# anonymousauthors001/SGS-GNN

Measured on AMD Instinct MI355X. Metric: sampled edges/sec + training steps/sec, Reddit hybrid 20% sparsity, higher is better.
Workload: dtype f32

## Files before the change

include/sgs_hip.h:

```cpp
#ifndef SGS_HIP_H_
#define SGS_HIP_H_

#include <stddef.h>
#include <stdint.h>

#ifdef __cplusplus
extern "C" {
#endif

#define SGS_ABI_VERSION 1

#define SGS_OK 0
#define SGS_EINVAL (-1)
#define SGS_EWORKSPACE (-2)
#define SGS_EHIP (-3)

typedef void* sgs_stream_t;

int sgs_abi_version(void);
const char* sgs_last_error(void);

int sgs_rng_set_epoch_buffer(const uint64_t* epoch_dev);
int sgs_exp_noise(uint64_t seed, uint64_t stream_id, int64_t E, float* noise, sgs_stream_t stream);
int sgs_dropout_keep(uint64_t seed, uint32_t site, int64_t rows, int64_t cols, float p, uint8_t* keep,
// ... 8 lines not shown
#define SGS_SAMPLE_PRIOR 1

size_t sgs_sample_topq_workspace_bytes(int64_t E);
int sgs_sample_topq(int mode, const float* p, const float* prior, double degree_bias_coef,
                    const float* noise, uint64_t seed, uint64_t stream_id, int64_t E, int64_t q,
                    const int64_t* edge_index, uint8_t* mask, int64_t* sampled_eid,
                    int64_t* sampled_edge_index, float* sampled_p, float* stats, float* keys_out,
                    void* ws, size_t ws_bytes, sgs_stream_t stream);

size_t sgs_sample_topq_cover_workspace_bytes(int64_t E, int64_t N);
int sgs_sample_topq_cover_variant(int64_t N, int64_t E);
int sgs_sample_topq_cover(int mode, const float* p, const float* prior, double degree_bias_coef, const float* noise,
                          uint64_t seed, uint64_t stream_id, int64_t E, int64_t q, const int64_t* edge_index,
                          int64_t N, const int32_t* in_ptr, const int32_t* in_src, const int32_t* in_eid,
                          uint8_t* mask, int64_t* sampled_eid, int64_t* sampled_edge_index, float* sampled_p,
                          float* stats, float* keys_out, int32_t* cover_info, void* ws, size_t ws_bytes, sgs_stream_t stream);

int sgs_gather_columns(const int64_t* edge_index, int64_t E, const int64_t* idx, int64_t q, int64_t* out, sgs_stream_t stream);

size_t sgs_sampler_shard_workspace_bytes(int64_t E_local);
int64_t sgs_sampler_chunk(void);
int sgs_sampler_shard_partials(int stage, const float* p, int64_t E, const float* scal, float* part, sgs_stream_t stream);
int sgs_sampler_shard_finalize(int stage, const float* part_all, int64_t nblk_all, float* scal, sgs_stream_t stream);
int sgs_sampler_shard_keys(int mode, const float* p, const float* prior, double degree_bias_coef, const float* noise,
                           uint64_t seed, uint64_t stream_id, int64_t edge_offset, int64_t E, const float* scal,
                           uint32_t* keys, float* keys_out, uint32_t* hist, sgs_stream_t stream);
int sgs_sampler_shard_hist(const uint32_t* keys, int64_t E, int pass, const void* state, uint32_t* hist,
                           sgs_stream_t stream);
int sgs_sampler_select(uint32_t* hist, int pass, int64_t q, void* state, sgs_stream_t stream);
int sgs_sampler_shard_count(const uint32_t* keys, int64_t E, const void* state, uint32_t* counts, void* ws,
                            size_t ws_bytes, sgs_stream_t stream);
int sgs_sampler_shard_compact(const uint32_t* keys, int64_t E, const void* state, int64_t ties_local, int64_t q_local,
                              int64_t edge_offset, const float* p, const int64_t* edge_index_local, uint8_t* mask,
                              int64_t* sampled_eid, int64_t* sampled_edge_index, float* sampled_p, void* ws,
                              size_t ws_bytes, sgs_stream_t stream);

int sgs_st_weights_fwd(const float* p, const float* prior, double degree_bias_coef, const float* stats,
                       const int64_t* sampled_eid, int64_t E, int64_t q, float* w, sgs_stream_t stream);
size_t sgs_st_weights_bwd_workspace_bytes(int64_t E, int64_t q);
int sgs_st_weights_bwd(const float* p, const float* prior, double degree_bias_coef, const float* stats,
                       const int64_t* sampled_eid, const float* grad_w, int64_t E, int64_t q, float* grad_p,
                       void* ws, size_t ws_bytes, sgs_stream_t stream);

size_t sgs_graph_build_workspace_bytes(int64_t n_edges, int64_t N);
int sgs_graph_build(const int64_t* edge_index, int64_t n_edges, int64_t N, int32_t* in_ptr, int32_t* in_src,
                    int32_t* in_eid, int32_t* out_ptr, int32_t* out_dst, int32_t* out_eid, int32_t* loop_eid,
                    void* ws, size_t ws_bytes, sgs_stream_t stream);

size_t sgs_graph_filter_workspace_bytes(int64_t E_parent, int64_t N);
int sgs_graph_filter(const int32_t* pin_ptr, const int32_t* pin_src, const int32_t* pin_eid, const int32_t* pout_ptr,
                     const int32_t* pout_dst, const int32_t* pout_eid, int64_t E_parent, int64_t N, const uint8_t* mask,
                     const int64_t* sampled_eid, int64_t q, int32_t* in_ptr, int32_t* in_src, int32_t* in_eid, int32_t* out_ptr,
                     int32_t* out_dst, int32_t* out_eid, int32_t* loop_eid, void* ws, size_t ws_bytes, sgs_stream_t stream);

size_t sgs_graph_build_src_sorted_workspace_bytes(int64_t n_edges, int64_t N);
int sgs_graph_build_src_sorted(const int64_t* edge_index, int64_t n_edges, int64_t N, int32_t* in_ptr, int32_t* in_src, int32_t* in_eid,
                               int32_t* out_ptr, int32_t* out_dst, int32_t* out_eid, int32_t* loop_eid, int32_t* unsorted, void* ws,
                               size_t ws_bytes, sgs_stream_t stream);

int sgs_gcn_norm_fwd(const float* w, int64_t n_edges, int64_t N, const int32_t* in_ptr, const int32_t* in_src,
                     const int32_t* in_eid, const int32_t* out_ptr, const int32_t* out_dst, const int32_t* out_eid,
                     const int32_t* loop_eid, float* dis, float* loopw, float* what_in, float* what_out,
                     float* what_loop, sgs_stream_t stream);

int sgs_gcn_degree_partial(const float* w, int64_t n_edges, int64_t N, const int32_t* in_ptr, const int32_t* in_src,
                           const int32_t* in_eid, float* degpart, sgs_stream_t stream);
int sgs_gcn_norm_from_degree(const float* w, const float* degsum, int64_t n_edges, int64_t N, const int32_t* in_ptr,
                             const int32_t* in_src, const int32_t* in_eid, const int32_t* out_ptr,
                             const int32_t* out_dst, const int32_t* out_eid, float* dis, float* loopw, float* what_in,
                             float* what_out, float* what_loop, sgs_stream_t stream);
int sgs_bias_act(const float* X, const float* bias, int64_t N, int64_t D, int act, float p_drop, uint64_t seed,
                 uint32_t site, float* Y, sgs_stream_t stream);
int sgs_bias_act_rows(const float* X, const float* bias, int64_t n_rows, int64_t D, int64_t row_offset, int act, float p_drop,
                      uint64_t seed, uint32_t site, float* Y, sgs_stream_t stream);

int sgs_mean_weights(int64_t n_edges, int64_t N, const int32_t* in_ptr, const int32_t* out_ptr, const int32_t* out_dst,
                     float* what_in, float* what_out, sgs_stream_t stream);
int sgs_degree_prior_logits(const int64_t* edge_index, int64_t E, int64_t N, const int32_t* in_ptr,
                            const int32_t* out_ptr, float* logits, sgs_stream_t stream);

size_t sgs_gcn_norm_bwd_workspace_bytes(int64_t N);
int sgs_gcn_norm_bwd(const float* w, const float* gw_hat, const float* gloop, int64_t n_edges, int64_t N,
                     const float* dis, const float* loopw, const int32_t* in_ptr, const int32_t* in_src,
                     const int32_t* in_eid, const int32_t* out_ptr, const int32_t* out_dst, const int32_t* out_eid,
                     const int32_t* loop_eid, const int64_t* edge_index, float* dw, void* ws, size_t ws_bytes,
                     sgs_stream_t stream);
int sgs_gcn_norm_bwd_sum(const float* w, const float* gw_hat, const float* gloop, const float* gw_hat2, const float* gloop2, const float* dw_add,
                         int64_t n_edges, int64_t N, const float* dis, const float* loopw, const int32_t* in_ptr, const int32_t* in_src,
                         const int32_t* in_eid, const int32_t* out_ptr, const int32_t* out_dst, const int32_t* out_eid,
                         const int32_t* loop_eid, const int64_t* edge_index, float* dw, void* ws, size_t ws_bytes, sgs_stream_t stream);

int sgs_gcn_norm_bwd_node(const float* w, const float* gw_hat, const float* gloop, int64_t n_edges, int64_t N,
                          const float* dis, const float* loopw, const int32_t* in_ptr, const int32_t* in_src,
                          const int32_t* in_eid, const int32_t* out_ptr, const int32_t* out_dst, const int32_t* out_eid,
                          float* Hn, sgs_stream_t stream);
int sgs_gcn_norm_bwd_edge(const float* gw_hat, const float* gloop, int64_t n_edges, int64_t N, const float* dis,
                          const int32_t* loop_eid, const int64_t* edge_index, const float* Hn, float* dw,
                          sgs_stream_t stream);

#define SGS_ACT_NONE 0
#define SGS_ACT_RELU 1
#define SGS_ACT_RELU_DROPOUT 2
int sgs_spmm_csr(const float* X, int64_t N, int64_t D, int64_t nnz, const int32_t* ptr, const int32_t* col, const float* val,
                 const float* diag, const float* bias, int act, float p_drop, uint64_t seed, uint32_t site, float* Y,
                 sgs_stream_t stream);

int sgs_sddmm_csr(const float* A, const float* B, int64_t N, int64_t D, int64_t nnz, const int32_t* ptr, const int32_t* col,
                  const int32_t* eid, float* g, float* gdiag, sgs_stream_t stream);

int sgs_spmm_csr_variant(int64_t N, int64_t D, int64_t nnz, int aligned16);
int sgs_sddmm_csr_variant(int64_t N, int64_t D, int64_t nnz, int aligned16);

int sgs_spmm_long_rows_set(int on);
int sgs_spmm_long_rows_threshold(void);
int sgs_spmm_long_rows_active(int64_t N, int64_t D);

// ... 90 lines not shown
                                    float* out_codes, float* out_U, float* out_U_raw, sgs_stream_t stream);
int sgs_edge_score_bwd_prep_sd_pack(const float* codes, int64_t N, int64_t H, const int64_t* edge_index, int64_t E, const int64_t* active_eid,
                                    int64_t n_active, const float* grad_p, const float* p, const uint32_t* maskbits, float* dz, uint32_t* dvbits,
                                    int32_t* sd, const float* W1, const float* w2, float p_drop, void* ws, size_t ws_bytes, sgs_stream_t stream);
int sgs_edge_score_bwd_dfeat_fused_packed(const uint32_t* dvbits, const float* dz, const int32_t* sd, const float* codes, int64_t n, int64_t N,
                                          int64_t H, float* G, float* opart, const void* ws, size_t ws_bytes, sgs_stream_t stream);
int sgs_edge_score_bwd_core_bits(const float* codes, const float* U, int64_t N, int64_t H, const int64_t* edge_index, int64_t E,
                                 int64_t edge_id_offset, const int64_t* active_eid, int64_t n_active, const float* grad_p, const float* W1,
                                 const float* b1, const float* w2, const float* b2, float p_drop, uint64_t seed, uint32_t site,
                                 uint32_t* dvbits, float* hdz_part, float* dz, float* feat, void* ws, size_t ws_bytes, sgs_stream_t stream);
int sgs_edge_score_bwd_dfeat_bits(const uint32_t* dvbits, const float* dz, int64_t n, int64_t H, const float* W1, const float* w2, float p_drop,
                                  float* dfeat, void* ws, size_t ws_bytes, sgs_stream_t stream);
int sgs_endpoint_reduce_pair_bits(const float* dfeat, const uint32_t* dvbits, const float* dz, const float* w2, float p_drop, const float* codes,
                                  int64_t N, int64_t H, int64_t nnz, const int32_t* in_ptr, const int32_t* in_src, const int32_t* in_eid,
                                  const int32_t* out_ptr, const int32_t* out_dst, const int32_t* out_eid, float* out_codes, float* out_U,
                                  float* out_U_raw, sgs_stream_t stream);
int sgs_gemm_tn_mask_supported(int64_t K, int64_t M, int64_t N);
int sgs_gemm_tn_mask_gather(const uint32_t* Abits, const float* dz, const float* rowscale, float scale, const float* codes, int64_t codes_rows,
                            const int32_t* sd, int64_t K, int64_t M, int64_t N, float* C, int64_t ldc, float* colsum_A, float* dz_sum, float* C_raw,
                            float* colsum_raw, void* ws, size_t ws_bytes, sgs_stream_t stream);
void sgs_gemm_tn_set_gather_variant(int shared, int slabs);
int sgs_gemm_tn_mask(const uint32_t* Abits, const float* dz, const float* rowscale, float scale, const float* B, int64_t K, int64_t M, int64_t N,
                     float* C, int64_t ldc, float* colsum_A, float* dz_sum, float* C_raw, float* colsum_raw, void* ws, size_t ws_bytes,
                     sgs_stream_t stream);

int sgs_edge_score_bf16_supported(int64_t H);
int sgs_edge_score_fwd_bf16(const float* codes, const float* U, int64_t N, int64_t H, const int64_t* edge_index, int64_t E,
                            int64_t edge_id_offset, const float* W1, const float* b1, const float* w2, const float* b2, float p_drop,
                            uint64_t seed, uint32_t site, float* p_out, void* ws, size_t ws_bytes, sgs_stream_t stream);
int sgs_edge_score_fwd_paired_bf16(const float* codes, const float* U, int64_t N, int64_t H, const int64_t* edge_index, int64_t E,
                                   int64_t edge_id_offset, const int32_t* canon, int64_t M, const int32_t* mate, const float* W1, const float* b1,
                                   const float* w2, const float* b2, float p_drop, uint64_t seed, uint32_t site, float* p_out, void* ws,
                                   size_t ws_bytes, sgs_stream_t stream);
int sgs_edge_score_fwd_mask_bf16(const float* codes, const float* U, int64_t N, int64_t H, const int64_t* edge_index, int64_t E,
                                 int64_t edge_id_offset, const int32_t* canon, int64_t M, const int32_t* mate, const float* W1, const float* b1,
                                 const float* w2, const float* b2, float p_drop, uint64_t seed, uint32_t site, float* p_out, uint32_t* maskbits,
                                 void* ws, size_t ws_bytes, sgs_stream_t stream);
int sgs_edge_score_bwd_dfeat_bits_bf16(const uint32_t* dvbits, const float* dz, int64_t n, int64_t H, const float* W1, const float* w2,
                                       float p_drop, float* dfeat, void* ws, size_t ws_bytes, sgs_stream_t stream);
int sgs_edge_score_bwd_prep_sd_pack_bf16(const float* codes, int64_t N, int64_t H, const int64_t* edge_index, int64_t E, const int64_t* active_eid,
                                         int64_t n_active, const float* grad_p, const float* p, const uint32_t* maskbits, float* dz, uint32_t* dvbits,
                                         int32_t* sd, const float* W1, const float* w2, float p_drop, void* ws, size_t ws_bytes, sgs_stream_t stream);
int sgs_edge_score_bwd_dfeat_fused_bf16(const uint32_t* dvbits, const float* dz, const int32_t* sd, const float* codes, int64_t n, int64_t N,
                                        int64_t H, const float* W1, const float* w2, float p_drop, float* G, float* opart, void* ws, size_t ws_bytes,
                                        sgs_stream_t stream);
int sgs_edge_score_bwd_dfeat_fused_packed_bf16(const uint32_t* dvbits, const float* dz, const int32_t* sd, const float* codes, int64_t n, int64_t N,
                                               int64_t H, float* G, float* opart, const void* ws, size_t ws_bytes, sgs_stream_t stream);
int sgs_gemm_tn_mask_bf16(const uint32_t* Abits, const float* dz, const float* rowscale, float scale, const float* B, int64_t K, int64_t M, int64_t N,
                          float* C, int64_t ldc, float* colsum_A, float* dz_sum, float* C_raw, float* colsum_raw, void* ws, size_t ws_bytes,
                          sgs_stream_t stream);
int sgs_gemm_tn_mask_gather_bf16(const uint32_t* Abits, const float* dz, const float* rowscale, float scale, const float* codes, int64_t codes_rows,
                                 const int32_t* sd, int64_t K, int64_t M, int64_t N, float* C, int64_t ldc, float* colsum_A, float* dz_sum, float* C_raw,
                                 float* colsum_raw, void* ws, size_t ws_bytes, sgs_stream_t stream);

int sgs_endpoint_reduce(const float* M_out, const float* M_in, const float* T, int64_t N, int64_t H, int64_t nnz,
                        const int32_t* in_ptr, const int32_t* in_src, const int32_t* in_eid, const int32_t* out_ptr,
                        const int32_t* out_dst, const int32_t* out_eid, float sign_out, float sign_in, float* out,
                        sgs_stream_t stream);
int sgs_endpoint_reduce_pair(const float* dfeat, const float* dv, const float* codes, int64_t N, int64_t H, int64_t nnz,
                             const int32_t* in_ptr, const int32_t* in_src, const int32_t* in_eid, const int32_t* out_ptr,
                             const int32_t* out_dst, const int32_t* out_eid, float* out_codes, float* out_U, sgs_stream_t stream);

int sgs_masked_correct(const float* logits, int64_t N, int64_t C, const int64_t* y, const uint8_t* train_mask,
                       int32_t* correct, sgs_stream_t stream);
int sgs_masked_correct_pair(const float* logits_a, const float* logits_b, int64_t N, int64_t C, const int64_t* y,
                            const uint8_t* train_mask, int32_t* correct4, sgs_stream_t stream);

int sgs_confusion_counts(const float* logits, int64_t N, int64_t C, const int64_t* y, const uint8_t* m0, const uint8_t* m1, const uint8_t* m2,
                         int64_t* conf, sgs_stream_t stream);
int sgs_confusion_variant(int64_t N, int64_t C);
int sgs_confusion_variant_set(int code);

size_t sgs_gate_counts_workspace_bytes(int64_t N);
int sgs_gate_counts(const float* logits_a, const float* logits_b, int64_t N, int64_t C, const int64_t* y, const uint8_t* train_mask,
                    int32_t* out5, const uint64_t* seq_dev, int32_t* dst_host_mapped, void* ws, size_t ws_bytes, sgs_stream_t stream);

int sgs_loss_tick(float* loss_sum, const float* loss, uint64_t* epoch, sgs_stream_t stream);
int sgs_publish_to_host(const int32_t* src_dev, int64_t n, const uint64_t* seq_dev, int32_t* dst_host_mapped, sgs_stream_t stream);

int sgs_masked_ce_fwd(const float* logits, int64_t N, int64_t C, const int64_t* y, const uint8_t* train_mask,
                      float* loss, float* row_lse, float* rowloss, int32_t* n_rows, sgs_stream_t stream);
int sgs_masked_ce_bwd(const float* logits, int64_t N, int64_t C, const int64_t* y, const uint8_t* train_mask,
                      const float* row_lse, const int32_t* n_rows, const float* grad_loss, float* dlogits,
                      sgs_stream_t stream);

size_t sgs_edge_reg_workspace_bytes(int64_t q);
int sgs_edge_reg_fwd(const float* w, const int64_t* sampled_edge_index, int64_t q, const float* logits, int64_t N,
                     int64_t C, const int64_t* y, const uint8_t* train_mask, float coef1, float coef2, float* out,
                     float* cos_out, void* ws, size_t ws_bytes, sgs_stream_t stream);
int sgs_edge_reg_bwd(const float* w, const int64_t* sampled_edge_index, int64_t q, int64_t q_global, const float* logits,
                     int64_t N, int64_t C, const int64_t* y, const uint8_t* train_mask, const float* out, float coef1,
                     float coef2, const float* grad_loss, float* dw, float* Gs, float* Gd, sgs_stream_t stream);

int sgs_hybrid_loss_fwd(const float* logits, int64_t N, int64_t C, const int64_t* y, const uint8_t* train_mask, const float* w,
                        const int64_t* sampled_edge_index, int64_t q, float coef1, float coef2, float* out, float* row_lse, float* rowloss,
                        int32_t* n_rows, void* ws, size_t ws_bytes, sgs_stream_t stream);
int sgs_masked_ce_bwd_acc(const float* logits, int64_t N, int64_t C, const int64_t* y, const uint8_t* train_mask, const float* row_lse,
                          const int32_t* n_rows, const float* grad_loss, float* dlogits, sgs_stream_t stream);

int sgs_masked_ce_w_fwd(const float* logits, int64_t N, int64_t C, const int64_t* y, const uint8_t* train_mask, const float* weight,
                        float label_smoothing, float* loss, float* row_lse, float* rowloss, float* den, sgs_stream_t stream);
int sgs_masked_ce_w_bwd(const float* logits, int64_t N, int64_t C, const int64_t* y, const uint8_t* train_mask, const float* weight,
                        float label_smoothing, const float* row_lse, const float* den, const float* grad_loss, float* dlogits,
                        sgs_stream_t stream);
int sgs_masked_ce_w_bwd_acc(const float* logits, int64_t N, int64_t C, const int64_t* y, const uint8_t* train_mask, const float* weight,
                            float label_smoothing, const float* row_lse, const float* den, const float* grad_loss, float* dlogits,
// ... 208 lines not shown
```

sgs-gnn_amd/csrc/edge_score.hip:

```cpp
#include <type_traits>

#include "sgs_common.h"
#include "endpoint_reduce.h"

namespace sgs {
namespace {

constexpr int kT = 256;
constexpr int kBM = 64;
constexpr int kBK = 16;
using f32x16 = __attribute__((ext_vector_type(16))) float;

__global__ void __launch_bounds__(kT) transpose_w1a(const float* __restrict__ W1, int H, float* __restrict__ WaT) {
    __shared__ float t[32][33];
    const int bx = blockIdx.x * 32, by = blockIdx.y * 32;
    const int tx = threadIdx.x & 31, ty = threadIdx.x >> 5;
    for (int r = ty; r < 32; r += 8) {
        const int h = by + r, k = bx + tx;
        t[r][tx] = (h < H && k < H) ? W1[static_cast<int64_t>(h) * 2 * H + k] : 0.f;
    }
    __syncthreads();
    for (int r = ty; r < 32; r += 8) {
        const int k = bx + r, h = by + tx;
        if (k < H && h < H) WaT[static_cast<int64_t>(k) * H + h] = t[tx][r];
    }
}

__global__ void __launch_bounds__(kT) transpose_w1_full(const float* __restrict__ W1, int H, float* __restrict__ WT) {
    __shared__ float t[32][33];
    const int bx = blockIdx.x * 32, by = blockIdx.y * 32;
    const int tx = threadIdx.x & 31, ty = threadIdx.x >> 5;
    for (int r = ty; r < 32; r += 8) {
        const int h = by + r, k = bx + tx;
        t[r][tx] = (h < H && k < 2 * H) ? W1[static_cast<int64_t>(h) * 2 * H + k] : 0.f;
    }
    __syncthreads();
    for (int r = ty; r < 32; r += 8) {
        const int k = bx + r, h = by + tx;
        if (k < 2 * H && h < H) WT[static_cast<int64_t>(k) * H + h] = t[tx][r];
    }
}

struct ScoreArgs {
    const float* codes;
    const float* U;
    const int64_t* src;
    const int64_t* dst;
    const int64_t* active;
    int64_t n;
    const int32_t* canon;
    const int32_t* mate;
    const int64_t* dyn_n;
    int64_t row_offset;
    int H;
    const float* WaT;
    const float* b1;
// ... 1738 lines not shown
                    ok[u] = k < total ? 1.f : 0.f;
                    sg[u] = k < total ? (isout ? 1.f : -1.f) : 0.f;
                }
                float m1[kEpU][4], m2[kEpU][4], t[kEpU][4];
                uint32_t wd[kEpU];
                float dzr[kEpU];
#pragma unroll
                for (int u = 0; u < kEpU; ++u) {
                    *reinterpret_cast<float4*>(m1[u]) = *reinterpret_cast<const float4*>(dfeat + static_cast<int64_t>(er[u]) * H + c0);
                    *reinterpret_cast<float4*>(t[u]) = *reinterpret_cast<const float4*>(codes + static_cast<int64_t>(cr[u]) * H + c0);
                    if constexpr (BITS) {
                        wd[u] = bits[static_cast<int64_t>(er[u]) * (H >> 5) + (c0 >> 5)];
                        dzr[u] = dz[er[u]];
                    } else {
                        *reinterpret_cast<float4*>(m2[u]) = *reinterpret_cast<const float4*>(dv + static_cast<int64_t>(er[u]) * H + c0);
                    }
                }
#pragma unroll
                for (int u = 0; u < kEpU; ++u) {
                    if constexpr (BITS) {
                        const uint32_t w = wd[u] >> (c0 & 31);
#pragma unroll
                        for (int j = 0; j < 4; ++j) m2[u][j] = (w >> j) & 1u ? dzr[u] : 0.f;
                    }
#pragma unroll
                    for (int j = 0; j < 4; ++j) {
                        a1[j] = fmaf(ok[u] * m1[u][j], t[u][j], a1[j]);
                        a2[j] = fmaf(sg[u], m2[u][j], a2[j]);
                    }
                }
            }
        }
#pragma unroll
        for (int j = 0; j < 4; ++j) { part[0][wave][lane * 4 + j] = a1[j]; part[1][wave][lane * 4 + j] = a2[j]; }
        __syncthreads();
        for (int tt = threadIdx.x; tt < 512; tt += 64 * NW) {
            const int which = tt >> 8, c = tt & 255;
            if (cbase + c < H) {
                float sum = 0.f;
#pragma unroll
                for (int g = 0; g < NW; g += 4) sum += (part[which][g][c] + part[which][g + 1][c]) + (part[which][g + 2][c] + part[which][g + 3][c]);
                if (BITS && which) {
                    if (out_Uraw) out_Uraw[v * H + cbase + c] = sum;
                    sum *= w2[cbase + c] * scale;
                }
                (which ? out_U : out_codes)[v * H + cbase + c] = sum;
            }
        }
        __syncthreads();
    }
}

template <int NW>
__global__ void __launch_bounds__(64 * NW) scorer_bwd_reduce(const float* __restrict__ G, const float* __restrict__ opart,
                                                            const uint32_t* __restrict__ bits, const float* __restrict__ dz,
                                                            const float* __restrict__ w2, float scale, int64_t N, int64_t H,
                                                            const int* __restrict__ in_ptr, const int* __restrict__ in_eid,
                                                            const int* __restrict__ out_ptr, float* __restrict__ out_codes,
                                                            float* __restrict__ out_U, float* __restrict__ out_Uraw) {
    __shared__ float part[2][NW][256];
    const int lane = threadIdx.x & 63, wave = threadIdx.x >> 6;
    const int64_t v = blockIdx.x;
    const int ob = out_ptr[v], no = out_ptr[v + 1] - ob;
    const int ib = in_ptr[v], ni = in_ptr[v + 1] - ib;
    const int w0 = ob >> 5, np = no > 0 ? ((ob + no - 1) >> 5) - w0 + 1 : 0;
    const int wpr = static_cast<int>(H >> 5);
    for (int64_t cbase = 0; cbase < H; cbase += 256) {
        const int64_t c0 = cbase + static_cast<int64_t>(lane) * 4;
        float a1[4] = {0.f, 0.f, 0.f, 0.f}, a2[4] = {0.f, 0.f, 0.f, 0.f};
        if (c0 < H) {
            const int wsel = static_cast<int>(c0 >> 5), wsh = static_cast<int>(c0 & 31);
            for (int k0 = wave; k0 < ni; k0 += kEpU * NW) {
                int er[kEpU];
                float ok[kEpU];
#pragma unroll
                for (int u = 0; u < kEpU; ++u) {
                    const int k = k0 + NW * u;
                    er[u] = in_eid[ib + (k < ni ? k : ni - 1)];
                    ok[u] = k < ni ? 1.f : 0.f;
                }
                float4 m1[kEpU];
                uint32_t wd[kEpU];
                float dzr[kEpU];
#pragma unroll
                for (int u = 0; u < kEpU; ++u) {
                    m1[u] = *reinterpret_cast<const float4*>(G + static_cast<int64_t>(er[u]) * H + c0);
                    wd[u] = bits[static_cast<int64_t>(er[u]) * wpr + wsel];
                    dzr[u] = dz[er[u]];
                }
#pragma unroll
                for (int u = 0; u < kEpU; ++u) {
                    const uint32_t w = wd[u] >> wsh;
                    const float dd = ok[u] * dzr[u];
                    a1[0] = fmaf(ok[u], m1[u].x, a1[0]); a1[1] = fmaf(ok[u], m1[u].y, a1[1]);
                    a1[2] = fmaf(ok[u], m1[u].z, a1[2]); a1[3] = fmaf(ok[u], m1[u].w, a1[3]);
#pragma unroll
                    for (int j = 0; j < 4; ++j) a2[j] -= (w >> j) & 1u ? dd : 0.f;
                }
            }
            for (int k0 = wave; k0 < no; k0 += kEpU * NW) {
                uint32_t wd[kEpU];
                float dzr[kEpU];
#pragma unroll
                for (int u = 0; u < kEpU; ++u) {
                    const int k = k0 + NW * u;
                    const int64_t e = ob + (k < no ? k : no - 1);
                    wd[u] = bits[e * wpr + wsel];
                    dzr[u] = dz[e] * (k < no ? 1.f : 0.f);
                }
#pragma unroll
                for (int u = 0; u < kEpU; ++u) {
                    const uint32_t w = wd[u] >> wsh;
#pragma unroll
                    for (int j = 0; j < 4; ++j) a2[j] += (w >> j) & 1u ? dzr[u] : 0.f;
                }
            }
            for (int k0 = wave; k0 < np; k0 += kEpU * NW) {
                float4 m1[kEpU];
                float ok[kEpU];
#pragma unroll
                for (int u = 0; u < kEpU; ++u) {
                    const int k = k0 + NW * u;
                    const int64_t slot = static_cast<int64_t>(w0 + (k < np ? k : np - 1)) + v;
                    m1[u] = *reinterpret_cast<const float4*>(opart + slot * H + c0);
                    ok[u] = k < np ? 1.f : 0.f;
                }
#pragma unroll
                for (int u = 0; u < kEpU; ++u) {
                    a1[0] = fmaf(ok[u], m1[u].x, a1[0]); a1[1] = fmaf(ok[u], m1[u].y, a1[1]);
                    a1[2] = fmaf(ok[u], m1[u].z, a1[2]); a1[3] = fmaf(ok[u], m1[u].w, a1[3]);
                }
            }
        }
#pragma unroll
        for (int j = 0; j < 4; ++j) { part[0][wave][lane * 4 + j] = a1[j]; part[1][wave][lane * 4 + j] = a2[j]; }
        __syncthreads();
        for (int tt = threadIdx.x; tt < 512; tt += 64 * NW) {
            const int which = tt >> 8, c = tt & 255;
            if (cbase + c < H) {
                float sum = 0.f;
#pragma unroll
                for (int g = 0; g < NW; g += 4) sum += (part[which][g][c] + part[which][g + 1][c]) + (part[which][g + 2][c] + part[which][g + 3][c]);
                if (which) {
                    if (out_Uraw) out_Uraw[v * H + cbase + c] = sum;
                    sum *= w2[cbase + c] * scale;
                }
                (which ? out_U : out_codes)[v * H + cbase + c] = sum;
            }
        }
        __syncthreads();
    }
}

__global__ void __launch_bounds__(256) epd_endpoint_reduce(const float* __restrict__ dfeat2, const float* __restrict__ A, int64_t N, int64_t H,
                                                          const int* __restrict__ in_ptr, const int* __restrict__ in_src,
                                                          const int* __restrict__ in_eid, const int* __restrict__ out_ptr,
                                                          const int* __restrict__ out_dst, const int* __restrict__ out_eid,
                                                          const int64_t* __restrict__ active, int64_t row_offset, uint64_t seed_x, uint32_t site_x,
                                                          uint64_t seed_y, uint32_t site_y, const uint64_t* __restrict__ epoch, uint32_t thresh,
                                                          float scale, int use_drop, float* __restrict__ dA) {
    constexpr int NW = 4;
    __shared__ float part[NW][256];
    const int lane = threadIdx.x & 63, wave = threadIdx.x >> 6;
    const int64_t v = blockIdx.x;
    const int ob = out_ptr[v], no = out_ptr[v + 1] - ob;
    const int ib = in_ptr[v], ni = in_ptr[v + 1] - ib;
    const int total = no + ni;
    const uint64_t sx = fold_epoch(seed_x, epoch), sy = fold_epoch(seed_y, epoch);
    for (int64_t cbase = 0; cbase < H; cbase += 256) {
        const int64_t c0 = cbase + static_cast<int64_t>(lane) * 4;
        float acc[4] = {0.f, 0.f, 0.f, 0.f};
        if (c0 < H) {
            for (int k = wave; k < total; k += NW) {
                const bool isout = k < no;
                const int idx = isout ? ob + k : ib + (k - no);
                const int r = (isout ? out_eid : in_eid)[idx];
                const int o = (isout ? out_dst : in_src)[idx];
                const int64_t e = row_offset + (active ? active[r] : static_cast<int64_t>(r));
                const float4 fa = *reinterpret_cast<const float4*>(dfeat2 + static_cast<int64_t>(r) * 2 * H + c0);
                const float4 fb = *reinterpret_cast<const float4*>(dfeat2 + static_cast<int64_t>(r) * 2 * H + H + c0);
                const float4 ao = *reinterpret_cast<const float4*>(A + static_cast<int64_t>(o) * H + c0);
                float ko[4] = {1.f, 1.f, 1.f, 1.f}, km[4] = {1.f, 1.f, 1.f, 1.f};
                if (use_drop) {
                    const uint32_t rx = dropout_row_key(sx, site_x, static_cast<uint64_t>(e)), ry = dropout_row_key(sy, site_y, static_cast<uint64_t>(e));
                    const uint32_t rmine = isout ? rx : ry, rother = isout ? ry : rx;
                    const uint32_t m0 = dropout_pair_bits(rmine, static_cast<uint32_t>(c0 >> 1)), m1 = dropout_pair_bits(rmine, static_cast<uint32_t>((c0 >> 1) + 1));
                    const uint32_t o0 = dropout_pair_bits(rother, static_cast<uint32_t>(c0 >> 1)), o1 = dropout_pair_bits(rother, static_cast<uint32_t>((c0 >> 1) + 1));
                    km[0] = (m0 & 0xFFFFu) >= thresh ? scale : 0.f; km[1] = (m0 >> 16) >= thresh ? scale : 0.f;
                    km[2] = (m1 & 0xFFFFu) >= thresh ? scale : 0.f; km[3] = (m1 >> 16) >= thresh ? scale : 0.f;
                    ko[0] = (o0 & 0xFFFFu) >= thresh ? scale : 0.f; ko[1] = (o0 >> 16) >= thresh ? scale : 0.f;
                    ko[2] = (o1 & 0xFFFFu) >= thresh ? scale : 0.f; ko[3] = (o1 >> 16) >= thresh ? scale : 0.f;
                }
                const float fav[4] = {fa.x, fa.y, fa.z, fa.w}, fbv[4] = {fb.x, fb.y, fb.z, fb.w}, aov[4] = {ao.x, ao.y, ao.z, ao.w};
                const float sg = isout ? 1.f : -1.f;
#pragma unroll
                for (int j = 0; j < 4; ++j) acc[j] += (fav[j] * (aov[j] * ko[j]) + sg * fbv[j]) * km[j];
            }
        }
#pragma unroll
        for (int j = 0; j < 4; ++j) part[wave][lane * 4 + j] = acc[j];
        __syncthreads();
        const int tt = threadIdx.x;
        if (cbase + tt < H) dA[v * H + cbase + tt] = (part[0][tt] + part[1][tt]) + (part[2][tt] + part[3][tt]);
        __syncthreads();
// ... 570 lines not shown
    if (n == 0) return SGS_OK;
    SGS_REQUIRE(dvbits && dz && sd && codes && (packed || (W1 && w2)) && G && opart, SGS_EINVAL, "%s: null pointer", who);
    SGS_REQUIRE(ws && ws_bytes >= sgs_edge_score_workspace_bytes(0, H, 0), SGS_EWORKSPACE, "%s: workspace too small", who);
    uint4* const Wp16 = fused_wp16(ws, H);
    if (!packed) launch_pack_w1a<true>(P, W1, H, Wp16, stream, w2, 1.0f / (1.0f - p_drop));
    ScoreArgs a{};
    a.inbits = dvbits; a.indz = dz; a.n = n; a.H = static_cast<int>(H); a.feat = G; a.codes = codes; a.sd = sd; a.opart = opart;
    return P == 1 ? launch_bf16x6<5, 1>(a, Wp16, n, H, stream) : launch_bf16x6<5, 3>(a, Wp16, n, H, stream);
}

int sgs_edge_score_bwd_dfeat_fused(const uint32_t* dvbits, const float* dz, const int32_t* sd, const float* codes, int64_t n, int64_t N, int64_t H,
                                   const float* W1, const float* w2, float p_drop, float* G, float* opart, void* ws, size_t ws_bytes,
                                   sgs_stream_t stream_) {
    return bwd_dfeat_fused_impl("sgs_edge_score_bwd_dfeat_fused", 3, sgs_edge_score_bwd_bits_supported, false, dvbits, dz, sd, codes, n, N, H, W1, w2,
                                p_drop, G, opart, ws, ws_bytes, stream_);
}

int sgs_edge_score_bwd_dfeat_fused_packed(const uint32_t* dvbits, const float* dz, const int32_t* sd, const float* codes, int64_t n, int64_t N,
                                          int64_t H, float* G, float* opart, const void* ws, size_t ws_bytes, sgs_stream_t stream_) {
    return bwd_dfeat_fused_impl("sgs_edge_score_bwd_dfeat_fused_packed", 3, sgs_edge_score_bwd_bits_supported, true, dvbits, dz, sd, codes, n, N, H,
                                nullptr, nullptr, 0.f, G, opart, const_cast<void*>(ws), ws_bytes, stream_);
}

int sgs_edge_score_bwd_dfeat_fused_bf16(const uint32_t* dvbits, const float* dz, const int32_t* sd, const float* codes, int64_t n, int64_t N,
                                        int64_t H, const float* W1, const float* w2, float p_drop, float* G, float* opart, void* ws, size_t ws_bytes,
                                        sgs_stream_t stream_) {
    return bwd_dfeat_fused_impl("sgs_edge_score_bwd_dfeat_fused_bf16", 1, sgs_edge_score_bf16_supported, false, dvbits, dz, sd, codes, n, N, H, W1, w2,
                                p_drop, G, opart, ws, ws_bytes, stream_);
}

int sgs_edge_score_bwd_dfeat_fused_packed_bf16(const uint32_t* dvbits, const float* dz, const int32_t* sd, const float* codes, int64_t n, int64_t N,
                                               int64_t H, float* G, float* opart, const void* ws, size_t ws_bytes, sgs_stream_t stream_) {
    return bwd_dfeat_fused_impl("sgs_edge_score_bwd_dfeat_fused_packed_bf16", 1, sgs_edge_score_bf16_supported, true, dvbits, dz, sd, codes, n, N, H,
                                nullptr, nullptr, 0.f, G, opart, const_cast<void*>(ws), ws_bytes, stream_);
}

int sgs_edge_score_bwd_reduce_fused(const float* G, const float* opart, const uint32_t* dvbits, const float* dz, const float* w2, float p_drop,
                                    int64_t N, int64_t H, int64_t nnz, const int32_t* in_ptr, const int32_t* in_eid, const int32_t* out_ptr,
                                    float* out_codes, float* out_U, float* out_U_raw, sgs_stream_t stream_) {
    hipStream_t stream = static_cast<hipStream_t>(stream_);
    SGS_REQUIRE(N >= 0 && H >= 0 && H % 32 == 0 && N < (int64_t(1) << 31) && p_drop >= 0.f && p_drop < 1.f, SGS_EINVAL,
                "sgs_edge_score_bwd_reduce_fused: needs H %% 32 == 0");
    if (N == 0 || H == 0) return SGS_OK;
    SGS_REQUIRE(G && opart && dvbits && dz && w2 && in_ptr && in_eid && out_ptr && out_codes && out_U, SGS_EINVAL,
                "sgs_edge_score_bwd_reduce_fused: null pointer");
    const dim3 grid(static_cast<unsigned>(N));
    const float scale = 1.0f / (1.0f - p_drop);
    SGS_LAUNCH_ROWBLOCK((scorer_bwd_reduce<16>), (scorer_bwd_reduce<4>), G, opart, dvbits, dz, w2, scale, N, H, in_ptr, in_eid, out_ptr, out_codes,
                        out_U, out_U_raw);
    SGS_LAUNCH_OK();
    return SGS_OK;
}

int sgs_edge_score_dw2_from_parts(const float* W1, const float* T_raw, const float* U, const float* R_raw, const float* b1, const float* c_raw,
                                  int64_t N, int64_t H, float p_drop, float* dw2, sgs_stream_t stream_) {
    hipStream_t stream = static_cast<hipStream_t>(stream_);
    SGS_REQUIRE(N > 0 && H > 0 && p_drop >= 0.f && p_drop < 1.f && W1 && T_raw && U && R_raw && b1 && c_raw && dw2, SGS_EINVAL,
                "sgs_edge_score_dw2_from_parts: bad arguments");
    hipLaunchKernelGGL(scorer_dw2_from_parts, dim3(static_cast<unsigned>(H)), dim3(kT), 0, stream, W1, T_raw, U, R_raw, b1, c_raw, N,
                       static_cast<int>(H), 1.0f / (1.0f - p_drop), dw2);
    SGS_LAUNCH_OK();
    return SGS_OK;
}

int sgs_endpoint_reduce_pair_bits(const float* dfeat, const uint32_t* dvbits, const float* dz, const float* w2, float p_drop, const float* codes,
                                  int64_t N, int64_t H, int64_t nnz, const int32_t* in_ptr, const int32_t* in_src, const int32_t* in_eid,
                                  const int32_t* out_ptr, const int32_t* out_dst, const int32_t* out_eid, float* out_codes, float* out_U,
                                  float* out_U_raw, sgs_stream_t stream_) {
    hipStream_t stream = static_cast<hipStream_t>(stream_);
    SGS_REQUIRE(N >= 0 && H >= 0 && H % 32 == 0 && N < (int64_t(1) << 31) && p_drop >= 0.f && p_drop < 1.f, SGS_EINVAL,
                "sgs_endpoint_reduce_pair_bits: needs H %% 32 == 0");
    if (N == 0 || H == 0) return SGS_OK;
    SGS_REQUIRE(dfeat && dvbits && dz && w2 && codes && in_ptr && out_ptr && out_codes && out_U, SGS_EINVAL,
                "sgs_endpoint_reduce_pair_bits: null pointer");
    const dim3 grid(static_cast<unsigned>(N));
    const float scale = 1.0f / (1.0f - p_drop);
    const float* nodv = nullptr;
    SGS_LAUNCH_ROWBLOCK((endpoint_reduce_pair_rowblock<16, true>), (endpoint_reduce_pair_rowblock<4, true>), dfeat, nodv, codes, N, H, in_ptr, in_src,
                        in_eid, out_ptr, out_dst, out_eid, out_codes, out_U, dvbits, dz, w2, scale, out_U_raw);
    SGS_LAUNCH_OK();
    return SGS_OK;
}

size_t sgs_edge_score_epd_workspace_bytes(int64_t H) { return carve_bytes(2 * static_cast<size_t>(H < 0 ? 0 : H) * (H < 0 ? 0 : H), 4) + 256; }

static int epd_args(ScoreArgs& a, const char* who, const float* A, int64_t N, int64_t H, const int64_t* edge_index, int64_t E, const int64_t* active,
                    int64_t n, int64_t edge_id_offset, const float* W1, const float* b1, const float* w2, const float* b2, float p_hidden, uint64_t seed,
                    uint32_t site, float p_ep,
                    uint64_t seed_x, uint32_t site_x, uint64_t seed_y, uint32_t site_y, void* ws, size_t ws_bytes, hipStream_t stream) {
    if (int rc = check_common(who, N, H, E, p_hidden)) return rc;
    SGS_REQUIRE(H % 16 == 0, SGS_EINVAL, "%s: the endpoint-dropout scorer needs H %% 16 == 0 (H=%lld)", who, (long long)H);
    SGS_REQUIRE(p_ep >= 0.f && p_ep < 1.f, SGS_EINVAL, "%s: bad endpoint dropout probability", who);
    SGS_REQUIRE(A && edge_index && W1 && b1 && w2 && b2, SGS_EINVAL, "%s: null pointer", who);
    SGS_REQUIRE(ws && ws_bytes >= sgs_edge_score_epd_workspace_bytes(H), SGS_EWORKSPACE, "%s: workspace too small", who);
    Carver cv(ws);
    float* WT = cv.take<float>(2 * static_cast<size_t>(H) * H);
    hipLaunchKernelGGL(transpose_w1_full, dim3(cdiv(2 * H, 32), cdiv(H, 32)), dim3(kT), 0, stream, W1, static_cast<int>(H), WT);
    score_args(a, A, nullptr, edge_index, E, active, n, edge_id_offset, H, WT, b1, w2, b2, p_hidden, seed, site);
    a.epd = p_ep > 0.f; a.seed_x = seed_x; a.seed_y = seed_y; a.site_x = site_x; a.site_y = site_y;
    a.ep_scale = 1.0f / (1.0f - p_ep); a.ep_thresh = dropout_thresh(p_ep);
    return SGS_OK;
}

int sgs_edge_score_epd_fwd(const float* A, int64_t N, int64_t H, const int64_t* edge_index, int64_t E, int64_t edge_id_offset, const float* W1,
                           const float* b1, const float* w2, const float* b2, float p_hidden, uint64_t seed, uint32_t site, float p_ep,
                           uint64_t seed_x, uint32_t site_x, uint64_t seed_y, uint32_t site_y, float* p_out, void* ws, size_t ws_bytes,
// ... 57 lines not shown
```

sgs-gnn_amd/csrc/gcn.hip:

```cpp
#include "sgs_common.h"

namespace sgs {
size_t graph_sort_workspace_bytes(int64_t n, int64_t N);
size_t graph_src_sorted_workspace_bytes(int64_t n, int64_t N);
int graph_build_src_sorted(const int64_t* ei, int64_t n, int64_t N, int32_t* in_ptr, int32_t* in_src, int32_t* in_eid, int32_t* out_ptr,
                           int32_t* out_dst, int32_t* out_eid, int32_t* loop_eid, int32_t* unsorted_flag, void* ws, size_t ws_bytes,
                           hipStream_t stream);
int graph_build_by_sort(const int64_t* ei, int64_t n, int64_t N, int32_t* in_ptr, int32_t* in_src, int32_t* in_eid, int32_t* out_ptr,
                        int32_t* out_dst, int32_t* out_eid, int32_t* loop_eid, void* ws, size_t ws_bytes, hipStream_t stream);
}

namespace sgs {
namespace {

constexpr int kT = 256;
constexpr int kMaxLdsRow = 8192;

__global__ void __launch_bounds__(kT) count_degrees(const int64_t* __restrict__ ei, int64_t n_edges, int* __restrict__ cnt_in,
                                                   int* __restrict__ cnt_out, int* __restrict__ loop_eid) {
    const int64_t e = static_cast<int64_t>(blockIdx.x) * kT + threadIdx.x;
    if (e >= n_edges) return;
    const int s = static_cast<int>(ei[e]), d = static_cast<int>(ei[n_edges + e]);
    atomicAdd(&cnt_in[d], 1);
    atomicAdd(&cnt_out[s], 1);
// ... 213 lines not shown
        if (e < E && mask[e]) v |= 1u << j;
    }
    bits[w] = v;
}
template <bool BITS>
__device__ __forceinline__ bool mask_at(const uint8_t* __restrict__ mask, int e) {
    if (BITS) return (reinterpret_cast<const uint32_t*>(mask)[e >> 5] >> (e & 31)) & 1u;
    return mask[e] != 0;
}

template <bool BITS>
__device__ __forceinline__ void filter_count_scatter_body(const int* __restrict__ in_ptr, const int* __restrict__ in_eid,
                                                          const int* __restrict__ out_ptr, const int* __restrict__ out_eid, int64_t N,
                                                          const uint8_t* __restrict__ mask, const int64_t* __restrict__ sampled_eid,
                                                          int64_t q, int64_t n_row_blocks, int* __restrict__ cnt_in,
                                                          int* __restrict__ cnt_out, int* __restrict__ pos, int64_t nrows) {
    if (static_cast<int64_t>(blockIdx.x) >= n_row_blocks) {
        const int64_t j = (static_cast<int64_t>(blockIdx.x) - n_row_blocks) * kT + threadIdx.x;
        if (j < q) pos[sampled_eid[j]] = static_cast<int>(j);
        return;
    }
    const int lane = threadIdx.x & 63;
    const int64_t r = (static_cast<int64_t>(blockIdx.x) * kT + threadIdx.x) >> 6;
    if (r >= nrows) return;
    const bool out = r >= N;
    const int64_t row = out ? r - N : r;
    const int* ptr = out ? out_ptr : in_ptr;
    const int* eid = out ? out_eid : in_eid;
    int c = 0;
    const int b = ptr[row], e = ptr[row + 1];
    for (int k = b + lane; k < e; k += 256) {
        int id[4];
#pragma unroll
        for (int u = 0; u < 4; ++u) id[u] = eid[min(k + 64 * u, e - 1)];
#pragma unroll
        for (int u = 0; u < 4; ++u) {
            const bool m = mask_at<BITS>(mask, id[u]);
            c += (k + 64 * u < e && m) ? 1 : 0;
        }
    }
    c = wave_sum_int_all(c);
    if (lane == 0) (out ? cnt_out : cnt_in)[row] = c;
}
template <bool BITS>
__global__ void __launch_bounds__(kT) filter_count_scatter(const int* __restrict__ in_ptr, const int* __restrict__ in_eid,
                                                          const int* __restrict__ out_ptr, const int* __restrict__ out_eid, int64_t N,
                                                          const uint8_t* __restrict__ mask, const int64_t* __restrict__ sampled_eid,
                                                          int64_t q, int64_t n_row_blocks, int* __restrict__ cnt_in,
                                                          int* __restrict__ cnt_out, int* __restrict__ pos) {
    filter_count_scatter_body<BITS>(in_ptr, in_eid, out_ptr, out_eid, N, mask, sampled_eid, q, n_row_blocks, cnt_in, cnt_out, pos, 2 * N);
}

constexpr int64_t kSelfScanRows = 4096;
template <bool BITS, bool SCAN>
__device__ __forceinline__ void filter_fill_body(int64_t nrows, const int* __restrict__ pin_ptr, const int* __restrict__ pin_src, const int* __restrict__ pin_eid,
                                                 const int* __restrict__ pout_ptr, const int* __restrict__ pout_dst,
                                                 const int* __restrict__ pout_eid, int64_t N, const uint8_t* __restrict__ mask,
                                                 const int* __restrict__ pos, int* __restrict__ in_ptr, int* __restrict__ in_src,
                                                 int* __restrict__ in_eid, int* __restrict__ out_ptr, int* __restrict__ out_dst,
                                                 int* __restrict__ out_eid, int* __restrict__ loop_eid, const int* __restrict__ cnt_in,
                                                 const int* __restrict__ cnt_out) {
    const int lane = threadIdx.x & 63;
    const int64_t r = (static_cast<int64_t>(blockIdx.x) * kT + threadIdx.x) >> 6;
    if (r >= nrows) return;
    const bool out = r >= N;
    const int64_t row = out ? r - N : r;
    const int* pptr = out ? pout_ptr : pin_ptr;
    const int* pcol = out ? pout_dst : pin_src;
    const int* peid = out ? pout_eid : pin_eid;
    int* ccol = out ? out_dst : in_src;
    int* ceid = out ? out_eid : in_eid;
    int w;
    if constexpr (SCAN) {
        const int* cnt = out ? cnt_out : cnt_in;
        int acc = 0;
        for (int64_t i = lane; i < row; i += 64) acc += cnt[i];
        w = wave_sum_int_all(acc);
        if (lane == 0) {
            int* cptr = out ? out_ptr : in_ptr;
            cptr[row] = w;
            if (row == N - 1) cptr[N] = w + cnt[row];
        }
    } else {
        w = (out ? out_ptr : in_ptr)[row];
    }
    int loop = -1;
    const int b = pptr[row], e = pptr[row + 1];
    int pe_c = 0, col_c = 0;
    if (e > b) { const int kc = min(b + lane, e - 1); pe_c = peid[kc]; col_c = pcol[kc]; }
    for (int k0 = b; k0 < e; k0 += 64) {
        const int k = k0 + lane;
        const int kn = min(k + 64, e - 1);
        const int pe_n = peid[kn], col_n = pcol[kn];
        const bool m_c = mask_at<BITS>(mask, pe_c);
        const bool sel = k < e && m_c;
        const int ne = sel ? pos[pe_c] : 0;
        const int col = col_c;
        pe_c = pe_n; col_c = col_n;
        const unsigned long long bal = __ballot(sel);
        if (sel) {
            const int o = w + __popcll(bal & ((1ull << lane) - 1ull));
            ccol[o] = col;
            ceid[o] = ne;
        }
        if (!out) {
            const unsigned long long lb = __ballot(sel && col == static_cast<int>(row));
            if (lb) loop = __shfl(ne, 63 - __clzll(lb), 64);
        }
        w += __popcll(bal);
    }
    if (!out && lane == 0) loop_eid[row] = loop;
}
template <bool BITS, bool SCAN = false>
__global__ void __launch_bounds__(kT) filter_fill(const int* __restrict__ pin_ptr, const int* __restrict__ pin_src, const int* __restrict__ pin_eid,
                                                 const int* __restrict__ pout_ptr, const int* __restrict__ pout_dst,
                                                 const int* __restrict__ pout_eid, int64_t N, const uint8_t* __restrict__ mask,
                                                 const int* __restrict__ pos, int* __restrict__ in_ptr, int* __restrict__ in_src,
                                                 int* __restrict__ in_eid, int* __restrict__ out_ptr, int* __restrict__ out_dst,
                                                 int* __restrict__ out_eid, int* __restrict__ loop_eid, const int* __restrict__ cnt_in = nullptr,
                                                 const int* __restrict__ cnt_out = nullptr) {
    filter_fill_body<BITS, SCAN>(2 * N, pin_ptr, pin_src, pin_eid, pout_ptr, pout_dst, pout_eid, N, mask, pos, in_ptr, in_src, in_eid, out_ptr,
                                 out_dst, out_eid, loop_eid, cnt_in, cnt_out);
}

__device__ __forceinline__ void norm_deg_body(const float* __restrict__ w, int64_t N, const int* __restrict__ in_ptr,
                                              const int* __restrict__ in_src, const int* __restrict__ in_eid,
                                              const int* __restrict__ loop_eid, float* __restrict__ dis,
                                              float* __restrict__ loopw) {
    const int lane = threadIdx.x & 63;
    const int64_t i = (static_cast<int64_t>(blockIdx.x) * kT + threadIdx.x) >> 6;
    if (i >= N) return;
    const int b = in_ptr[i], e = in_ptr[i + 1];
    float acc = 0.f;
    for (int k = b + lane; k < e; k += 64) {
        if (in_src[k] != static_cast<int>(i)) acc += w ? w[in_eid[k]] : 1.0f;
    }
    acc = wave_sum_all(acc);
    const int le = loop_eid[i];
    const float lw = (le >= 0 && w) ? w[le] : 1.0f;
    const float deg = lw + acc;
    float di = 1.0f / sqrtf(deg);
    if (isinf(di)) di = 0.f;
    if (lane == 0) { dis[i] = di; loopw[i] = lw; }
}
__global__ void __launch_bounds__(kT) norm_deg(const float* __restrict__ w, int64_t N, const int* __restrict__ in_ptr,
                                              const int* __restrict__ in_src, const int* __restrict__ in_eid,
                                              const int* __restrict__ loop_eid, float* __restrict__ dis,
                                              float* __restrict__ loopw) {
    norm_deg_body(w, N, in_ptr, in_src, in_eid, loop_eid, dis, loopw);
}

__global__ void __launch_bounds__(kT) deg_partial(const float* __restrict__ w, int64_t N, const int* __restrict__ in_ptr,
                                                 const int* __restrict__ in_src, const int* __restrict__ in_eid,
                                                 float* __restrict__ degpart) {
    const int lane = threadIdx.x & 63;
    const int64_t i = (static_cast<int64_t>(blockIdx.x) * kT + threadIdx.x) >> 6;
    if (i >= N) return;
    float acc = 0.f;
    for (int k = in_ptr[i] + lane; k < in_ptr[i + 1]; k += 64)
        if (in_src[k] != static_cast<int>(i)) acc += w ? w[in_eid[k]] : 1.0f;
    acc = wave_sum_all(acc);
    if (lane == 0) degpart[i] = acc;
}
__global__ void __launch_bounds__(kT) dis_from_degree(const float* __restrict__ degsum, int64_t N, float* __restrict__ dis,
                                                     float* __restrict__ loopw) {
    const int64_t i = static_cast<int64_t>(blockIdx.x) * kT + threadIdx.x;
    if (i >= N) return;
    float di = 1.0f / sqrtf(1.0f + degsum[i]);
    if (isinf(di)) di = 0.f;
    dis[i] = di;
    loopw[i] = 1.0f;
}
__global__ void __launch_bounds__(kT) bias_act(const float* __restrict__ X, const float* __restrict__ bias, int64_t N, int64_t D, int act,
                                              float drop_scale, uint32_t drop_thresh, uint64_t seed, uint32_t site,
                                              const uint64_t* __restrict__ epoch, float* __restrict__ Y, int64_t row_offset) {
    seed = fold_epoch(seed, epoch);
    const int64_t idx = static_cast<int64_t>(blockIdx.x) * kT + threadIdx.x;
    if (idx >= N * D) return;
    const int64_t i = idx / D;
    const uint32_t c = static_cast<uint32_t>(idx - i * D);
    float y = X[idx];
    if (bias) y += bias[c];
    if (act != SGS_ACT_NONE) y = fmaxf(y, 0.f);
    if (act == SGS_ACT_RELU_DROPOUT) y = dropout_keep_at(seed, site, static_cast<uint64_t>(row_offset + i), c, drop_thresh) ? y * drop_scale : 0.f;
    Y[idx] = y;
}

__global__ void __launch_bounds__(kT) mean_weights(int64_t N, const int* __restrict__ in_ptr, const int* __restrict__ out_ptr,
                                                  const int* __restrict__ out_dst, float* __restrict__ what_in,
                                                  float* __restrict__ what_out) {
    const int lane = threadIdx.x & 63;
    const int64_t r = (static_cast<int64_t>(blockIdx.x) * kT + threadIdx.x) >> 6;
    if (r >= 2 * N) return;
    if (r < N) {
        const int b = in_ptr[r], e = in_ptr[r + 1];
        const float w = e > b ? 1.0f / static_cast<float>(e - b) : 0.f;
        for (int k = b + lane; k < e; k += 64) what_in[k] = w;
    } else {
        const int64_t i = r - N;
        for (int k = out_ptr[i] + lane; k < out_ptr[i + 1]; k += 64) {
            const int t = out_dst[k];
            what_out[k] = 1.0f / static_cast<float>(in_ptr[t + 1] - in_ptr[t]);
// ... 952 lines not shown
}

size_t sgs_graph_filter_workspace_bytes(int64_t E_parent, int64_t N) {
    if (E_parent < 0) E_parent = 0;
    if (N < 0) N = 0;
    return 4 * carve_bytes(N + 1, 4) + carve_bytes(E_parent + 1, 4) + carve_bytes(E_parent / 32 + 2, 4) + 256;
}

int sgs_graph_filter(const int32_t* pin_ptr, const int32_t* pin_src, const int32_t* pin_eid, const int32_t* pout_ptr,
                     const int32_t* pout_dst, const int32_t* pout_eid, int64_t E_parent, int64_t N, const uint8_t* mask,
                     const int64_t* sampled_eid, int64_t q, int32_t* in_ptr, int32_t* in_src, int32_t* in_eid, int32_t* out_ptr,
                     int32_t* out_dst, int32_t* out_eid, int32_t* loop_eid, void* ws, size_t ws_bytes, sgs_stream_t stream_) {
    hipStream_t stream = static_cast<hipStream_t>(stream_);
    SGS_REQUIRE(E_parent >= 0 && N >= 0 && q >= 0 && q <= E_parent && E_parent < (int64_t(1) << 31) && N < (int64_t(1) << 30), SGS_EINVAL,
                "sgs_graph_filter: bad sizes");
    if (N == 0) return SGS_OK;
    SGS_REQUIRE(pin_ptr && pout_ptr && in_ptr && out_ptr && loop_eid && (E_parent == 0 || (pin_src && pin_eid && pout_dst && pout_eid && mask)) &&
                    (q == 0 || (sampled_eid && in_src && in_eid && out_dst && out_eid)), SGS_EINVAL, "sgs_graph_filter: null pointer");
    SGS_REQUIRE(ws && ws_bytes >= sgs_graph_filter_workspace_bytes(E_parent, N), SGS_EWORKSPACE, "sgs_graph_filter: workspace too small");
    Carver cv(ws);
    int* cnt_in = cv.take<int>(N + 1);
    int* cnt_out = cv.take<int>(N + 1);
    int* cur_in = cv.take<int>(N + 1);
    int* cur_out = cv.take<int>(N + 1);
    int* pos = cv.take<int>(E_parent + 1);
    uint32_t* bits = cv.take<uint32_t>(E_parent / 32 + 2);
    const int64_t n_row_blocks = cdiv(2 * N * 64, kT);
    const dim3 g1(static_cast<unsigned>(n_row_blocks + cdiv(q, kT))), g3(static_cast<unsigned>(n_row_blocks)), blk(kT);
    if (E_parent >= (int64_t(1) << 23)) {
        hipLaunchKernelGGL(pack_mask_bits, dim3(static_cast<unsigned>(cdiv(cdiv(E_parent, 32), kT))), blk, 0, stream, mask, E_parent, bits);
        const uint8_t* bm = reinterpret_cast<const uint8_t*>(bits);
        hipLaunchKernelGGL(filter_count_scatter<true>, g1, blk, 0, stream, pin_ptr, pin_eid, pout_ptr, pout_eid, N, bm, sampled_eid, q, n_row_blocks,
                           cnt_in, cnt_out, pos);
        hipLaunchKernelGGL(scan_counts, dim3(2), dim3(1024), 0, stream, cnt_in, cnt_out, N, in_ptr, out_ptr, cur_in, cur_out);
        hipLaunchKernelGGL(filter_fill<true>, g3, blk, 0, stream, pin_ptr, pin_src, pin_eid, pout_ptr, pout_dst, pout_eid, N, bm, pos, in_ptr, in_src,
                           in_eid, out_ptr, out_dst, out_eid, loop_eid);
    } else if (N <= kSelfScanRows) {
        hipLaunchKernelGGL(filter_count_scatter<false>, g1, blk, 0, stream, pin_ptr, pin_eid, pout_ptr, pout_eid, N, mask, sampled_eid, q,
                           n_row_blocks, cnt_in, cnt_out, pos);
        hipLaunchKernelGGL((filter_fill<false, true>), g3, blk, 0, stream, pin_ptr, pin_src, pin_eid, pout_ptr, pout_dst, pout_eid, N, mask, pos,
                           in_ptr, in_src, in_eid, out_ptr, out_dst, out_eid, loop_eid, static_cast<const int*>(cnt_in),
                           static_cast<const int*>(cnt_out));
    } else {
        hipLaunchKernelGGL(filter_count_scatter<false>, g1, blk, 0, stream, pin_ptr, pin_eid, pout_ptr, pout_eid, N, mask, sampled_eid, q,
                           n_row_blocks, cnt_in, cnt_out, pos);
        hipLaunchKernelGGL(scan_counts, dim3(2), dim3(1024), 0, stream, cnt_in, cnt_out, N, in_ptr, out_ptr, cur_in, cur_out);
        hipLaunchKernelGGL(filter_fill<false>, g3, blk, 0, stream, pin_ptr, pin_src, pin_eid, pout_ptr, pout_dst, pout_eid, N, mask, pos, in_ptr,
                           in_src, in_eid, out_ptr, out_dst, out_eid, loop_eid);
    }
    SGS_LAUNCH_OK();
    return SGS_OK;
}

size_t sgs_edge_mates_workspace_bytes(int64_t n_edges) { return carve_bytes(n_edges < 0 ? 0 : n_edges, 4) + 256; }

int sgs_edge_mates(const int64_t* edge_index, int64_t n_edges, int64_t N, const int32_t* out_ptr, const int32_t* out_dst,
                   const int32_t* out_eid, int32_t* mate, void* ws, size_t ws_bytes, sgs_stream_t stream_) {
    hipStream_t stream = static_cast<hipStream_t>(stream_);
    SGS_REQUIRE(n_edges >= 0 && N >= 0 && n_edges < (int64_t(1) << 31), SGS_EINVAL, "sgs_edge_mates: bad sizes");
    if (n_edges == 0) return SGS_OK;
    SGS_REQUIRE(edge_index && out_ptr && out_dst && out_eid && mate, SGS_EINVAL, "sgs_edge_mates: null pointer");
    SGS_REQUIRE(ws && ws_bytes >= sgs_edge_mates_workspace_bytes(n_edges), SGS_EWORKSPACE, "sgs_edge_mates: workspace too small");
    Carver cv(ws);
    int* rev = cv.take<int>(n_edges);
    const dim3 g(static_cast<unsigned>(cdiv(n_edges, kT))), blk(kT);
    hipLaunchKernelGGL(edge_reverse, g, blk, 0, stream, edge_index, n_edges, out_ptr, out_dst, out_eid, rev);
    hipLaunchKernelGGL(edge_mate, g, blk, 0, stream, rev, n_edges, mate);
    SGS_LAUNCH_OK();
    return SGS_OK;
}

int sgs_gcn_norm_fwd(const float* w, int64_t n_edges, int64_t N, const int32_t* in_ptr, const int32_t* in_src,
                     const int32_t* in_eid, const int32_t* out_ptr, const int32_t* out_dst, const int32_t* out_eid,
                     const int32_t* loop_eid, float* dis, float* loopw, float* what_in, float* what_out, float* what_loop,
                     sgs_stream_t stream_) {
    hipStream_t stream = static_cast<hipStream_t>(stream_);
    SGS_REQUIRE(N >= 0 && n_edges >= 0, SGS_EINVAL, "sgs_gcn_norm_fwd: bad sizes");
    if (N == 0) return SGS_OK;
    SGS_REQUIRE(in_ptr && out_ptr && loop_eid && dis && loopw && what_loop, SGS_EINVAL, "sgs_gcn_norm_fwd: null pointer");
    hipLaunchKernelGGL(norm_deg, dim3(cdiv(N * 64, kT)), dim3(kT), 0, stream, w, N, in_ptr, in_src, in_eid, loop_eid, dis, loopw);
    hipLaunchKernelGGL(norm_weights, dim3(cdiv(2 * N * 64, kT)), dim3(kT), 0, stream, w, N, n_edges, in_ptr, in_src, in_eid,
                       out_ptr, out_dst, out_eid, dis, loopw, what_in, what_out, what_loop);
    SGS_LAUNCH_OK();
    return SGS_OK;
}

int sgs_gcn_degree_partial(const float* w, int64_t n_edges, int64_t N, const int32_t* in_ptr, const int32_t* in_src,
                           const int32_t* in_eid, float* degpart, sgs_stream_t stream_) {
    hipStream_t stream = static_cast<hipStream_t>(stream_);
    SGS_REQUIRE(N >= 0 && n_edges >= 0, SGS_EINVAL, "sgs_gcn_degree_partial: bad sizes");
    if (N == 0) return SGS_OK;
    SGS_REQUIRE(in_ptr && degpart, SGS_EINVAL, "sgs_gcn_degree_partial: null pointer");
    hipLaunchKernelGGL(deg_partial, dim3(cdiv(N * 64, kT)), dim3(kT), 0, stream, w, N, in_ptr, in_src, in_eid, degpart);
    SGS_LAUNCH_OK();
    return SGS_OK;
}

int sgs_gcn_norm_from_degree(const float* w, const float* degsum, int64_t n_edges, int64_t N, const int32_t* in_ptr,
                             const int32_t* in_src, const int32_t* in_eid, const int32_t* out_ptr, const int32_t* out_dst,
                             const int32_t* out_eid, float* dis, float* loopw, float* what_in, float* what_out,
                             float* what_loop, sgs_stream_t stream_) {
    hipStream_t stream = static_cast<hipStream_t>(stream_);
    SGS_REQUIRE(N >= 0 && n_edges >= 0, SGS_EINVAL, "sgs_gcn_norm_from_degree: bad sizes");
    if (N == 0) return SGS_OK;
    SGS_REQUIRE(degsum && in_ptr && out_ptr && dis && loopw && what_loop, SGS_EINVAL, "sgs_gcn_norm_from_degree: null pointer");
    hipLaunchKernelGGL(dis_from_degree, dim3(cdiv(N, kT)), dim3(kT), 0, stream, degsum, N, dis, loopw);
    hipLaunchKernelGGL(norm_weights, dim3(cdiv(2 * N * 64, kT)), dim3(kT), 0, stream, w, N, n_edges, in_ptr, in_src, in_eid,
                       out_ptr, out_dst, out_eid, dis, loopw, what_in, what_out, what_loop);
    SGS_LAUNCH_OK();
    return SGS_OK;
}

int sgs_bias_act(const float* X, const float* bias, int64_t N, int64_t D, int act, float p_drop, uint64_t seed, uint32_t site,
                 float* Y, sgs_stream_t stream_) {
    return sgs_bias_act_rows(X, bias, N, D, 0, act, p_drop, seed, site, Y, stream_);
}

int sgs_bias_act_rows(const float* X, const float* bias, int64_t N, int64_t D, int64_t row_offset, int act, float p_drop, uint64_t seed,
                      uint32_t site, float* Y, sgs_stream_t stream_) {
    hipStream_t stream = static_cast<hipStream_t>(stream_);
    SGS_REQUIRE(N >= 0 && D >= 0 && D < (int64_t(1) << 32) && act >= SGS_ACT_NONE && act <= SGS_ACT_RELU_DROPOUT && p_drop >= 0.f &&
                    p_drop < 1.f, SGS_EINVAL, "sgs_bias_act: bad arguments");
    if (N * D == 0) return SGS_OK;
    SGS_REQUIRE(X && Y, SGS_EINVAL, "sgs_bias_act: null pointer");
    if (act == SGS_ACT_RELU_DROPOUT && p_drop == 0.f) act = SGS_ACT_RELU;
    hipLaunchKernelGGL(bias_act, dim3(cdiv(N * D, kT)), dim3(kT), 0, stream, X, bias, N, D, act, 1.0f / (1.0f - p_drop),
                       dropout_thresh(p_drop), seed, site, epoch_ptr(), Y, row_offset);
    SGS_LAUNCH_OK();
    return SGS_OK;
}

int sgs_mean_weights(int64_t n_edges, int64_t N, const int32_t* in_ptr, const int32_t* out_ptr, const int32_t* out_dst,
                     float* what_in, float* what_out, sgs_stream_t stream_) {
    hipStream_t stream = static_cast<hipStream_t>(stream_);
    SGS_REQUIRE(N >= 0 && n_edges >= 0, SGS_EINVAL, "sgs_mean_weights: bad sizes");
// ... 501 lines not shown
```

sgs-gnn_amd/csrc/gemm_tn.hip:

```cpp
#include "sgs_common.h"

namespace sgs {
namespace {

using f32x16 = __attribute__((ext_vector_type(16))) float;
constexpr int kUnroll = 8;

__global__ void __launch_bounds__(64) gemm_tn_tile(const float* __restrict__ A, const float* __restrict__ B, int64_t K, int M, int N,
                                                  int ksplit, float* __restrict__ slab) {
    const int lane = threadIdx.x, kh = lane >> 5, l31 = lane & 31;
    const int ti = blockIdx.x, tj = blockIdx.y, s = blockIdx.z;
    const int i = ti * 32 + l31, j = tj * 32 + l31;
    const bool iok = i < M, jok = j < N;
    const int64_t per = ((K + ksplit - 1) / ksplit + 1) & ~int64_t(1);
    const int64_t k0 = s * per, k1 = (k0 + per < K) ? k0 + per : K;
    f32x16 acc;
#pragma unroll
    for (int r = 0; r < 16; ++r) acc[r] = 0.f;
    int64_t k = k0;
    for (; k + 2 * kUnroll <= k1; k += 2 * kUnroll) {
        float a[kUnroll], b[kUnroll];
#pragma unroll
        for (int u = 0; u < kUnroll; ++u) {
            const int64_t kk = k + 2 * u + kh;
            a[u] = iok ? A[kk * M + i] : 0.f;
            b[u] = jok ? B[kk * N + j] : 0.f;
        }
#pragma unroll
        for (int u = 0; u < kUnroll; ++u) acc = __builtin_amdgcn_mfma_f32_32x32x2f32(a[u], b[u], acc, 0, 0, 0);
    }
    for (; k < k1; k += 2) {
        const int64_t kk = k + kh;
        const float a = (iok && kk < k1) ? A[kk * M + i] : 0.f;
        const float b = (jok && kk < k1) ? B[kk * N + j] : 0.f;
        acc = __builtin_amdgcn_mfma_f32_32x32x2f32(a, b, acc, 0, 0, 0);
    }
    float* out = slab + static_cast<int64_t>(s) * M * N;
    if (jok) {
#pragma unroll
        for (int r = 0; r < 16; ++r) {
            const int row = ti * 32 + (r & 3) + 8 * (r >> 2) + 4 * kh;
            if (row < M) out[static_cast<int64_t>(row) * N + j] = acc[r];
        }
    }
}

constexpr int kWgUnroll = 8;
template <int NW>
__device__ __forceinline__ void gemm_tn_wg_tile(const float* __restrict__ A, const float* __restrict__ B, int64_t K, int M, int N,
                                                float* __restrict__ C, int64_t ldc, int ti, int tj) {
    __shared__ float red[NW][16][64];
    const int lane = threadIdx.x & 63, s = threadIdx.x >> 6, kh = lane >> 5, l31 = lane & 31;
    const int i = ti * 32 + l31, j = tj * 32 + l31;
// ... 24 lines not shown
#pragma unroll
    for (int r = 0; r < 16; ++r) red[s][r][lane] = acc[r];
    __syncthreads();
    if (!jok) return;
    constexpr int RPW = 16 / NW;
#pragma unroll
    for (int q = 0; q < RPW; ++q) {
        const int r = s * RPW + q;
        float sum = 0.f;
#pragma unroll
        for (int z = 0; z < NW; ++z) sum += red[z][r][lane];
        const int row = ti * 32 + (r & 3) + 8 * (r >> 2) + 4 * kh;
        if (row < M) C[static_cast<int64_t>(row) * ldc + j] = sum;
    }
}

template <int NW>
__global__ void __launch_bounds__(64 * NW) gemm_tn_wg(const float* __restrict__ A, const float* __restrict__ B, int64_t K, int M, int N,
                                                     float* __restrict__ C, int64_t ldc) {
    gemm_tn_wg_tile<NW>(A, B, K, M, N, C, ldc, blockIdx.x, blockIdx.y);
}

constexpr int kGroupMax = 8;
struct GemmTnDesc {
    const float* A;
    const float* B;
    float* C;
    int64_t K, ldc;
    int M, N;
    int first_tile, tiles_i;
};
struct GemmTnGroupArgs {
    GemmTnDesc d[kGroupMax];
    int count;
};

template <int NW>
__global__ void __launch_bounds__(64 * NW) gemm_tn_wg_group(GemmTnGroupArgs a) {
    const int t = static_cast<int>(blockIdx.x);
    int pi = 0;
    while (pi + 1 < a.count && t >= a.d[pi + 1].first_tile) ++pi;
    const GemmTnDesc& d = a.d[pi];
    const int local = t - d.first_tile;
    const int tj = local / d.tiles_i, ti = local - tj * d.tiles_i;
    gemm_tn_wg_tile<NW>(d.A, d.B, d.K, d.M, d.N, d.C, d.ldc, ti, tj);
}

__global__ void __launch_bounds__(256) gemm_tn_reduce(const float* __restrict__ slab, int64_t mn, int ksplit, float* __restrict__ C,
                                                      const float* __restrict__ cpart = nullptr, int M = 0, float* __restrict__ colsum = nullptr,
                                                      int N = 0, int64_t ldc = 0, const float* __restrict__ rowscale = nullptr,
                                                      float scale = 1.f, const float* __restrict__ dzpart = nullptr, int nz = 0,
                                                      float* __restrict__ dzsum = nullptr, float* __restrict__ Craw = nullptr,
                                                      float* __restrict__ csraw = nullptr, int csplit = 0) {
    const int64_t i = static_cast<int64_t>(blockIdx.x) * 256 + threadIdx.x;
    if (i >= mn) {
        const int64_t c = i - mn;
        if (dzsum && c == M) {
            float acc = 0.f;
            for (int z = 0; z < nz; ++z) acc += dzpart[z];
            dzsum[0] = acc;
        }
        if (colsum && c < M) {
            float acc = 0.f;
            const int ncs = csplit > 0 ? csplit : ksplit;
            if (csplit > 0) {
                float a8[8] = {0.f, 0.f, 0.f, 0.f, 0.f, 0.f, 0.f, 0.f};
                int s = 0;
                for (; s + 8 <= ncs; s += 8) {
                    float v[8];
#pragma unroll
                    for (int j = 0; j < 8; ++j) v[j] = cpart[static_cast<int64_t>(s + j) * M + c];
#pragma unroll
                    for (int j = 0; j < 8; ++j) a8[j] += v[j];
                }
                for (; s < ncs; ++s) a8[0] += cpart[static_cast<int64_t>(s) * M + c];
                acc = ((a8[0] + a8[1]) + (a8[2] + a8[3])) + ((a8[4] + a8[5]) + (a8[6] + a8[7]));
            } else
            for (int s = 0; s < ncs; ++s) acc += cpart[static_cast<int64_t>(s) * M + c];
            if (csraw) csraw[c] = acc;
            colsum[c] = rowscale ? acc * (rowscale[c] * scale) : acc;
        }
        return;
    }
    float acc = 0.f;
    if (csplit > 0) {
        float a8[8] = {0.f, 0.f, 0.f, 0.f, 0.f, 0.f, 0.f, 0.f};
        int s = 0;
        for (; s + 8 <= ksplit; s += 8) {
            float v[8];
#pragma unroll
            for (int j = 0; j < 8; ++j) v[j] = slab[static_cast<int64_t>(s + j) * mn + i];
#pragma unroll
            for (int j = 0; j < 8; ++j) a8[j] += v[j];
        }
        for (; s < ksplit; ++s) a8[0] += slab[static_cast<int64_t>(s) * mn + i];
        acc = ((a8[0] + a8[1]) + (a8[2] + a8[3])) + ((a8[4] + a8[5]) + (a8[6] + a8[7]));
    } else
    for (int s = 0; s < ksplit; ++s) acc += slab[static_cast<int64_t>(s) * mn + i];
    if (Craw) Craw[i] = acc;
    if (rowscale) acc *= rowscale[i / N] * scale;
    if (ldc > 0 && ldc != N) C[(i / N) * ldc + (i % N)] = acc;
    else C[i] = acc;
}

constexpr int kTallK = 8192;
constexpr int kTallU = 8;

__global__ void __launch_bounds__(64) gemm_tn_tall_tile(const float* __restrict__ A, const float* __restrict__ B, int64_t K, int M, int N,
                                                       int ksplit, float* __restrict__ slab, float* __restrict__ cpart) {
    const int lane = threadIdx.x, kh = lane >> 5, l31 = lane & 31;
    const int m0 = blockIdx.x * 128, n0 = blockIdx.y * 64, s = blockIdx.z;
    const int ia = m0 + 4 * l31, jb = n0 + 2 * l31;
    const bool aok = ia < M, bok = jb < N;
    const int64_t per = ((K + ksplit - 1) / ksplit + 1) & ~int64_t(1);
    const int64_t k0 = s * per, k1 = (k0 + per < K) ? k0 + per : K;
    f32x16 acc[4][2];
#pragma unroll
    for (int t = 0; t < 4; ++t)
#pragma unroll
        for (int u = 0; u < 2; ++u)
#pragma unroll
            for (int r = 0; r < 16; ++r) acc[t][u][r] = 0.f;
    const float4 z4 = make_float4(0.f, 0.f, 0.f, 0.f);
    const float2 z2 = make_float2(0.f, 0.f);
    const bool want_cs = cpart != nullptr && blockIdx.y == 0;
    float cs[4] = {0.f, 0.f, 0.f, 0.f};
    auto load = [&](int64_t k, float4 (&a)[kTallU], float2 (&b)[kTallU]) {
#pragma unroll
        for (int u = 0; u < kTallU; ++u) {
            const int64_t kk = k + 2 * u + kh;
            const bool in = kk < k1;
            a[u] = (aok && in) ? *reinterpret_cast<const float4*>(A + kk * M + ia) : z4;
            b[u] = (bok && in) ? *reinterpret_cast<const float2*>(B + kk * N + jb) : z2;
        }
    };
    auto mma = [&](const float4 (&a)[kTallU], const float2 (&b)[kTallU]) {
#pragma unroll
        for (int u = 0; u < kTallU; ++u) {
            const float av[4] = {a[u].x, a[u].y, a[u].z, a[u].w};
            const float bv[2] = {b[u].x, b[u].y};
            if (want_cs) { cs[0] += av[0]; cs[1] += av[1]; cs[2] += av[2]; cs[3] += av[3]; }
#pragma unroll
            for (int t = 0; t < 4; ++t)
#pragma unroll
                for (int w = 0; w < 2; ++w) acc[t][w] = __builtin_amdgcn_mfma_f32_32x32x2f32(av[t], bv[w], acc[t][w], 0, 0, 0);
        }
    };
    float4 a0[kTallU], a1[kTallU];
    float2 b0[kTallU], b1[kTallU];
    load(k0, a0, b0);
#pragma unroll 1
    for (int64_t k = k0; k < k1; k += 4 * kTallU) {
        load(k + 2 * kTallU, a1, b1);
        mma(a0, b0);
        load(k + 4 * kTallU, a0, b0);
// ... 533 lines not shown
    for (int t = 0; t < MT; ++t)
#pragma unroll
        for (int r = 0; r < 16; ++r) {
            const int h = 32 * MT * w + MT * ((r & 3) + 8 * (r >> 2) + 4 * g) + t;
            *reinterpret_cast<float2*>(out + static_cast<int64_t>(h) * N + n0 + 2 * l31) = make_float2(acc[t][0][r], acc[t][1][r]);
        }
    if (want_cs && g == 0) {
        float* cp = cpart + (static_cast<int64_t>(slab_id) * NG + ng) * M + 32 * MT * w + MT * l31;
#pragma unroll
        for (int t = 0; t < MT; ++t) cp[t] = cs[t];
    }
}

constexpr int kMaskfeatMaxSlabs = 128;
inline bool use_tall(int64_t K, int64_t M, int64_t N) { return K >= kTallK && M % 4 == 0 && N % 2 == 0; }
inline int pick_ksplit_tall(int64_t K, int64_t M, int64_t N) {
    const int64_t tiles = cdiv(M, 128) * cdiv(N, 64);
    int ks = 1;
    while (ks < 512 && tiles * ks < 1024 && K / (ks * 2) >= 256) ks *= 2;
    return ks;
}

inline int pick_ksplit(int64_t K, int64_t M, int64_t N) {
    if (use_tall(K, M, N)) return pick_ksplit_tall(K, M, N);
    const int64_t tiles = cdiv(M, 32) * cdiv(N, 32);
    int ks = 1;
    while (ks < 64 && tiles * ks < 1024 && K / (ks * 2) >= 64) ks *= 2;
    return ks;
}

inline int wg_waves(int64_t K, int64_t M, int64_t N) {
    if (K <= 0 || M <= 0 || N <= 0 || use_tall(K, M, N)) return 0;
    const int ks = pick_ksplit(K, M, N);
    if (ks == 8 && K >= 512) return 16;
    return (ks == 2 || ks == 4 || ks == 8) ? ks : 0;
}

}
}

using namespace sgs;

extern "C" {

size_t sgs_gemm_tn_workspace_bytes(int64_t K, int64_t M, int64_t N) {
    if (K < 0 || M < 0 || N < 0) return 256;
    const size_t ks = static_cast<size_t>(pick_ksplit(K, M, N));
    return carve_bytes(ks * M * N, 4) + carve_bytes(ks * M, 4) + carve_bytes(kMaskfeatMaxSlabs * 8 * M + kMaskfeatMaxSlabs, 4) + 512;
}

static int gemm_tn_impl(const float* A, const float* B, int64_t K, int64_t M, int64_t N, float* C, float* colsum_A, void* ws,
                        size_t ws_bytes, hipStream_t stream, int64_t ldc = 0, const uint32_t* Abits = nullptr, const float* dz = nullptr,
                        const float* rowscale = nullptr, float scale = 1.f, float* dz_sum = nullptr, float* C_raw = nullptr,
                        float* colsum_raw = nullptr, const int32_t* sd = nullptr, bool one = false);
static int g_tall_bf16x6 = 1;
static int g_gather_shared = 1, g_gather_slabs = 0;
void sgs_gemm_tn_set_gather_variant(int shared, int slabs) { g_gather_shared = shared ? 1 : 0; g_gather_slabs = slabs > 0 ? slabs : 0; }
void sgs_gemm_tn_set_tall_variant(int v) { g_tall_bf16x6 = v < 0 ? 1 : (v ? 1 : 0); }

int sgs_gemm_tn(const float* A, const float* B, int64_t K, int64_t M, int64_t N, float* C, void* ws, size_t ws_bytes,
                sgs_stream_t stream_) {
    return gemm_tn_impl(A, B, K, M, N, C, nullptr, ws, ws_bytes, static_cast<hipStream_t>(stream_));
}

int sgs_gemm_tn_can_colsum(int64_t K, int64_t M, int64_t N) { return use_tall(K, M, N) && pick_ksplit_tall(K, M, N) > 1 ? 1 : 0; }

int sgs_gemm_tn_colsum(const float* A, const float* B, int64_t K, int64_t M, int64_t N, float* C, float* colsum_A, void* ws,
                       size_t ws_bytes, sgs_stream_t stream_) {
    SGS_REQUIRE(colsum_A && sgs_gemm_tn_can_colsum(K, M, N), SGS_EINVAL,
                "sgs_gemm_tn_colsum: shape not served by the tall-K kernel (check sgs_gemm_tn_can_colsum)");
    return gemm_tn_impl(A, B, K, M, N, C, colsum_A, ws, ws_bytes, static_cast<hipStream_t>(stream_));
}

int sgs_gemm_tn_ld(const float* A, const float* B, int64_t K, int64_t M, int64_t N, float* C, int64_t ldc, float* colsum_A, void* ws,
                   size_t ws_bytes, sgs_stream_t stream_) {
    SGS_REQUIRE(ldc >= N, SGS_EINVAL, "sgs_gemm_tn_ld: ldc < N");
    SGS_REQUIRE(!colsum_A || sgs_gemm_tn_can_colsum(K, M, N), SGS_EINVAL, "sgs_gemm_tn_ld: column sums only for the tall-K shapes");
    return gemm_tn_impl(A, B, K, M, N, C, colsum_A, ws, ws_bytes, static_cast<hipStream_t>(stream_), ldc);
}

int sgs_gemm_tn_mask_supported(int64_t K, int64_t M, int64_t N) {
    if (!use_tall(K, M, N) || M % 128 != 0 || N % 64 != 0) return 0;
    const int ks = pick_ksplit_tall(K, M, N);
    return (ks >= 4 && ks % 4 == 0) ? 1 : 0;
}

int sgs_gemm_tn_mask(const uint32_t* Abits, const float* dz, const float* rowscale, float scale, const float* B, int64_t K, int64_t M, int64_t N,
                     float* C, int64_t ldc, float* colsum_A, float* dz_sum, float* C_raw, float* colsum_raw, void* ws, size_t ws_bytes,
                     sgs_stream_t stream_) {
    SGS_REQUIRE(ldc >= N, SGS_EINVAL, "sgs_gemm_tn_mask: ldc < N");
    SGS_REQUIRE(Abits && dz && rowscale, SGS_EINVAL, "sgs_gemm_tn_mask: null pointer");
    SGS_REQUIRE(sgs_gemm_tn_mask_supported(K, M, N), SGS_EINVAL, "sgs_gemm_tn_mask: shape not served (check sgs_gemm_tn_mask_supported)");
    SGS_REQUIRE(!colsum_raw || colsum_A, SGS_EINVAL, "sgs_gemm_tn_mask: colsum_raw needs colsum_A");
    return gemm_tn_impl(nullptr, B, K, M, N, C, colsum_A, ws, ws_bytes, static_cast<hipStream_t>(stream_), ldc, Abits, dz, rowscale, scale, dz_sum,
                        C_raw, colsum_raw);
}

int sgs_gemm_tn_mask_gather(const uint32_t* Abits, const float* dz, const float* rowscale, float scale, const float* codes, int64_t codes_rows,
                            const int32_t* sd, int64_t K, int64_t M, int64_t N, float* C, int64_t ldc, float* colsum_A, float* dz_sum, float* C_raw,
                            float* colsum_raw, void* ws, size_t ws_bytes, sgs_stream_t stream_) {
    SGS_REQUIRE(ldc >= N, SGS_EINVAL, "sgs_gemm_tn_mask_gather: ldc < N");
    SGS_REQUIRE(codes_rows > 0 && codes_rows * N < (int64_t(1) << 32), SGS_EINVAL, "sgs_gemm_tn_mask_gather: the codes table needs 32-bit element offsets");
    SGS_REQUIRE(Abits && dz && rowscale && codes && sd, SGS_EINVAL, "sgs_gemm_tn_mask_gather: null pointer");
    SGS_REQUIRE(sgs_gemm_tn_mask_supported(K, M, N), SGS_EINVAL, "sgs_gemm_tn_mask_gather: shape not served (check sgs_gemm_tn_mask_supported)");
    SGS_REQUIRE(!colsum_raw || colsum_A, SGS_EINVAL, "sgs_gemm_tn_mask_gather: colsum_raw needs colsum_A");
    return gemm_tn_impl(nullptr, codes, K, M, N, C, colsum_A, ws, ws_bytes, static_cast<hipStream_t>(stream_), ldc, Abits, dz, rowscale, scale,
                        dz_sum, C_raw, colsum_raw, sd);
}

int sgs_gemm_tn_mask_bf16(const uint32_t* Abits, const float* dz, const float* rowscale, float scale, const float* B, int64_t K, int64_t M, int64_t N,
                          float* C, int64_t ldc, float* colsum_A, float* dz_sum, float* C_raw, float* colsum_raw, void* ws, size_t ws_bytes,
                          sgs_stream_t stream_) {
    SGS_REQUIRE(ldc >= N, SGS_EINVAL, "sgs_gemm_tn_mask_bf16: ldc < N");
    SGS_REQUIRE(Abits && dz && rowscale, SGS_EINVAL, "sgs_gemm_tn_mask_bf16: null pointer");
    SGS_REQUIRE(sgs_gemm_tn_mask_supported(K, M, N), SGS_EINVAL, "sgs_gemm_tn_mask_bf16: shape not served (check sgs_gemm_tn_mask_supported)");
    SGS_REQUIRE(!colsum_raw || colsum_A, SGS_EINVAL, "sgs_gemm_tn_mask_bf16: colsum_raw needs colsum_A");
    return gemm_tn_impl(nullptr, B, K, M, N, C, colsum_A, ws, ws_bytes, static_cast<hipStream_t>(stream_), ldc, Abits, dz, rowscale, scale, dz_sum,
                        C_raw, colsum_raw, nullptr, true);
}

int sgs_gemm_tn_mask_gather_bf16(const uint32_t* Abits, const float* dz, const float* rowscale, float scale, const float* codes, int64_t codes_rows,
                                 const int32_t* sd, int64_t K, int64_t M, int64_t N, float* C, int64_t ldc, float* colsum_A, float* dz_sum, float* C_raw,
                                 float* colsum_raw, void* ws, size_t ws_bytes, sgs_stream_t stream_) {
    SGS_REQUIRE(ldc >= N, SGS_EINVAL, "sgs_gemm_tn_mask_gather_bf16: ldc < N");
    SGS_REQUIRE(codes_rows > 0 && codes_rows * N < (int64_t(1) << 32), SGS_EINVAL,
                "sgs_gemm_tn_mask_gather_bf16: the codes table needs 32-bit element offsets");
    SGS_REQUIRE(Abits && dz && rowscale && codes && sd, SGS_EINVAL, "sgs_gemm_tn_mask_gather_bf16: null pointer");
    SGS_REQUIRE(sgs_gemm_tn_mask_supported(K, M, N), SGS_EINVAL, "sgs_gemm_tn_mask_gather_bf16: shape not served (check sgs_gemm_tn_mask_supported)");
    SGS_REQUIRE(!colsum_raw || colsum_A, SGS_EINVAL, "sgs_gemm_tn_mask_gather_bf16: colsum_raw needs colsum_A");
    return gemm_tn_impl(nullptr, codes, K, M, N, C, colsum_A, ws, ws_bytes, static_cast<hipStream_t>(stream_), ldc, Abits, dz, rowscale, scale,
                        dz_sum, C_raw, colsum_raw, sd, true);
}

static int gemm_tn_impl(const float* A, const float* B, int64_t K, int64_t M, int64_t N, float* C, float* colsum_A, void* ws,
                        size_t ws_bytes, hipStream_t stream, int64_t ldc, const uint32_t* Abits, const float* dz, const float* rowscale,
                        float scale, float* dz_sum, float* C_raw, float* colsum_raw, const int32_t* sd, bool one) {
    SGS_REQUIRE(K >= 0 && M >= 0 && N >= 0 && M < (1 << 30) && N < (1 << 30), SGS_EINVAL, "sgs_gemm_tn: bad sizes");
    if (M == 0 || N == 0) return SGS_OK;
    SGS_REQUIRE(C && (K == 0 || ((A || Abits) && B)), SGS_EINVAL, "sgs_gemm_tn: null pointer");
    SGS_REQUIRE(ws && ws_bytes >= sgs_gemm_tn_workspace_bytes(K, M, N), SGS_EWORKSPACE, "sgs_gemm_tn: workspace too small");
    const int ks = pick_ksplit(K, M, N);
    Carver cv(ws);
    float* slab = cv.take<float>(static_cast<size_t>(ks) * M * N);
    float* cpart = cv.take<float>(static_cast<size_t>(ks) * M);
    const bool strided = ldc > 0 && ldc != N;
    float* dst = (ks == 1 && !strided) ? C : slab;
    int n_slabs = ks;
    if (Abits) {
        constexpr int NW = 4;
        constexpr size_t lds = (NW / 2) * (128 * 64 + 4 * 64) * sizeof(float);
        static bool raised_m = false;
        if (!raised_m) {
            SGS_HIP_OK(hipFuncSetAttribute(reinterpret_cast<const void*>(&gemm_tn_tall_bf16x6<NW, true>), hipFuncAttributeMaxDynamicSharedMemorySize,
                                           static_cast<int>(lds)));
            raised_m = true;
        }
        n_slabs = ks / NW;
        float* dzpart = dz_sum ? cpart + static_cast<size_t>(n_slabs) * M : nullptr;
        const int NGc = static_cast<int>(N / 64);
        if (sd && g_gather_shared && (M == 128 || M == 256) && N % 64 == 0 && (NGc == 1 || NGc == 2 || NGc == 4 || NGc == 8) && K >= 64) {
            int ns = g_gather_slabs > 0 ? g_gather_slabs : 256 / NGc;
            while (ns > 1 && K / ns < 64) ns >>= 1;
            if (ns > kMaskfeatMaxSlabs) ns = kMaskfeatMaxSlabs;
            if (ns > ks) ns = ks;
            float* cpart2 = cv.take<float>(static_cast<size_t>(kMaskfeatMaxSlabs) * 8 * M + kMaskfeatMaxSlabs);
            float* dzp = dz_sum ? cpart2 + static_cast<size_t>(ns) * NGc * M : nullptr;
            const size_t lds_b = static_cast<size_t>(one ? maskfeat_lds_words(M / 128, 1) : 2 * 3 * (2 * 3 * 64 * 4 + (M / 32) * 16 + 16)) * 4;
            const dim3 grid(static_cast<unsigned>(NGc), static_cast<unsigned>(ns));
            float* cpa = (colsum_A || dz_sum) ? cpart2 : static_cast<float*>(nullptr);
            const int2* sd2 = reinterpret_cast<const int2*>(sd);
            const int Ni = static_cast<int>(N);
#define SGS_MASKFEAT(MT_, NG_)                                                                                                                 \
    do {                                                                                                                                       \
        if (one) hipLaunchKernelGGL((gemm_tn_maskfeat<MT_, NG_, 1>), grid, dim3(512), lds_b, stream, Abits, dz, B, sd2, K, Ni, slab, cpa, dzp);  \
        else     hipLaunchKernelGGL((gemm_tn_maskfeat<MT_, NG_>), grid, dim3(512), lds_b, stream, Abits, dz, B, sd2, K, Ni, slab, cpa, dzp);     \
    } while (0)
            if (M == 256) {
                if (NGc == 1) SGS_MASKFEAT(2, 1); else if (NGc == 2) SGS_MASKFEAT(2, 2); else if (NGc == 4) SGS_MASKFEAT(2, 4); else SGS_MASKFEAT(2, 8);
            } else {
                if (NGc == 1) SGS_MASKFEAT(1, 1); else if (NGc == 2) SGS_MASKFEAT(1, 2); else if (NGc == 4) SGS_MASKFEAT(1, 4); else SGS_MASKFEAT(1, 8);
            }
#undef SGS_MASKFEAT
            hipLaunchKernelGGL(gemm_tn_reduce, dim3(cdiv(M * N + M + 1, 256)), dim3(256), 0, stream, slab, M * N, ns, C,
                               static_cast<const float*>(colsum_A ? cpart2 : nullptr), static_cast<int>(M), colsum_A, static_cast<int>(N),
                               ldc > 0 ? ldc : N, rowscale, scale, static_cast<const float*>(dzp), ns, dz_sum, C_raw, colsum_raw, ns * NGc);
            SGS_LAUNCH_OK();
            return SGS_OK;
        }
        if (one) {
            static bool raised_1 = false;
            if (!raised_1) {
                SGS_HIP_OK(hipFuncSetAttribute(reinterpret_cast<const void*>(&gemm_tn_tall_bf16x6<NW, true, false, true>),
                                               hipFuncAttributeMaxDynamicSharedMemorySize, static_cast<int>(lds)));
                SGS_HIP_OK(hipFuncSetAttribute(reinterpret_cast<const void*>(&gemm_tn_tall_bf16x6<NW, true, true, true>),
                                               hipFuncAttributeMaxDynamicSharedMemorySize, static_cast<int>(lds)));
                raised_1 = true;
            }
            if (sd)
                hipLaunchKernelGGL((gemm_tn_tall_bf16x6<NW, true, true, true>), dim3(cdiv(M, 128), cdiv(N, 64), n_slabs), dim3(64 * NW), lds, stream, A, B,
                                   K, static_cast<int>(M), static_cast<int>(N), ks, slab, (colsum_A || dz_sum) ? cpart : static_cast<float*>(nullptr),
                                   Abits, dz, dzpart, sd);
            else
                hipLaunchKernelGGL((gemm_tn_tall_bf16x6<NW, true, false, true>), dim3(cdiv(M, 128), cdiv(N, 64), n_slabs), dim3(64 * NW), lds, stream, A,
                                   B, K, static_cast<int>(M), static_cast<int>(N), ks, slab, (colsum_A || dz_sum) ? cpart : static_cast<float*>(nullptr),
                                   Abits, dz, dzpart);
        } else if (sd) {
            static bool raised_g = false;
            if (!raised_g) {
                SGS_HIP_OK(hipFuncSetAttribute(reinterpret_cast<const void*>(&gemm_tn_tall_bf16x6<NW, true, true>),
                                               hipFuncAttributeMaxDynamicSharedMemorySize, static_cast<int>(lds)));
                raised_g = true;
            }
            hipLaunchKernelGGL((gemm_tn_tall_bf16x6<NW, true, true>), dim3(cdiv(M, 128), cdiv(N, 64), n_slabs), dim3(64 * NW), lds, stream, A, B, K,
                               static_cast<int>(M), static_cast<int>(N), ks, slab, (colsum_A || dz_sum) ? cpart : static_cast<float*>(nullptr), Abits,
                               dz, dzpart, sd);
        } else
        hipLaunchKernelGGL((gemm_tn_tall_bf16x6<NW, true>), dim3(cdiv(M, 128), cdiv(N, 64), n_slabs), dim3(64 * NW), lds, stream, A, B, K,
                           static_cast<int>(M), static_cast<int>(N), ks, slab, (colsum_A || dz_sum) ? cpart : static_cast<float*>(nullptr), Abits, dz,
                           dzpart);
        hipLaunchKernelGGL(gemm_tn_reduce, dim3(cdiv(M * N + M + 1, 256)), dim3(256), 0, stream, slab, M * N, n_slabs, C,
                           static_cast<const float*>(colsum_A ? cpart : nullptr), static_cast<int>(M), colsum_A, static_cast<int>(N),
                           ldc > 0 ? ldc : N, rowscale, scale, static_cast<const float*>(dzpart), ks, dz_sum, C_raw, colsum_raw);
        SGS_LAUNCH_OK();
        return SGS_OK;
    }
    if (use_tall(K, M, N) && g_tall_bf16x6 && ks >= 4 && ks % 4 == 0) {
        constexpr int NW = 4;
        constexpr size_t lds = (NW / 2) * (128 * 64 + 4 * 64) * sizeof(float);
        static bool raised = false;
        if (!raised) {
            SGS_HIP_OK(hipFuncSetAttribute(reinterpret_cast<const void*>(&gemm_tn_tall_bf16x6<NW>), hipFuncAttributeMaxDynamicSharedMemorySize,
                                           static_cast<int>(lds)));
            raised = true;
        }
        n_slabs = ks / NW;
        hipLaunchKernelGGL((gemm_tn_tall_bf16x6<NW>), dim3(cdiv(M, 128), cdiv(N, 64), n_slabs), dim3(64 * NW), lds, stream, A, B, K,
                           static_cast<int>(M), static_cast<int>(N), ks, slab, colsum_A ? cpart : static_cast<float*>(nullptr));
    } else if (use_tall(K, M, N) && g_tall_bf16x6)
        hipLaunchKernelGGL((gemm_tn_tall_bf16x6<1>), dim3(cdiv(M, 128), cdiv(N, 64), ks), dim3(64), 0, stream, A, B, K, static_cast<int>(M),
                           static_cast<int>(N), ks, dst, colsum_A ? cpart : static_cast<float*>(nullptr));
    else if (use_tall(K, M, N))
        hipLaunchKernelGGL(gemm_tn_tall_tile, dim3(cdiv(M, 128), cdiv(N, 64), ks), dim3(64), 0, stream, A, B, K, static_cast<int>(M),
                           static_cast<int>(N), ks, dst, colsum_A ? cpart : static_cast<float*>(nullptr));
    else if (const int nw = wg_waves(K, M, N)) {
        const dim3 grid(cdiv(M, 32), cdiv(N, 32));
        const int64_t ld = ldc > 0 ? ldc : N;
        if (nw == 16)     hipLaunchKernelGGL((gemm_tn_wg<16>), grid, dim3(1024), 0, stream, A, B, K, static_cast<int>(M), static_cast<int>(N), C, ld);
        else if (nw == 8) hipLaunchKernelGGL((gemm_tn_wg<8>), grid, dim3(512), 0, stream, A, B, K, static_cast<int>(M), static_cast<int>(N), C, ld);
        else if (nw == 4) hipLaunchKernelGGL((gemm_tn_wg<4>), grid, dim3(256), 0, stream, A, B, K, static_cast<int>(M), static_cast<int>(N), C, ld);
        else              hipLaunchKernelGGL((gemm_tn_wg<2>), grid, dim3(128), 0, stream, A, B, K, static_cast<int>(M), static_cast<int>(N), C, ld);
        SGS_LAUNCH_OK();
        return SGS_OK;
    } else
        hipLaunchKernelGGL(gemm_tn_tile, dim3(cdiv(M, 32), cdiv(N, 32), ks), dim3(64), 0, stream, A, B, K, static_cast<int>(M),
                           static_cast<int>(N), ks, dst);
    if (ks > 1 || strided)
        hipLaunchKernelGGL(gemm_tn_reduce, dim3(cdiv(M * N + (colsum_A ? M : 0), 256)), dim3(256), 0, stream, slab, M * N, n_slabs, C,
                           static_cast<const float*>(colsum_A ? cpart : nullptr), static_cast<int>(M), colsum_A, static_cast<int>(N), ldc);
    SGS_LAUNCH_OK();
    return SGS_OK;
}

int sgs_gemm_tn_group_supported(int64_t K, int64_t M, int64_t N) { return wg_waves(K, M, N); }

int sgs_gemm_tn_group(const SgsGemmTnProblem* problems, int count, sgs_stream_t stream_) {
    hipStream_t stream = static_cast<hipStream_t>(stream_);
    SGS_REQUIRE(count >= 0 && (count == 0 || problems), SGS_EINVAL, "sgs_gemm_tn_group: bad problem list");
    for (int p = 0; p < count; ++p) {
        const SgsGemmTnProblem& q = problems[p];
        SGS_REQUIRE(q.K >= 0 && q.M >= 0 && q.N >= 0 && q.M < (1 << 30) && q.N < (1 << 30), SGS_EINVAL, "sgs_gemm_tn_group: bad sizes");
        SGS_REQUIRE(q.ldc == 0 || q.ldc >= q.N, SGS_EINVAL, "sgs_gemm_tn_group: ldc < N");
        SGS_REQUIRE(q.M == 0 || q.N == 0 || (q.C && (q.K == 0 || (q.A && q.B))), SGS_EINVAL, "sgs_gemm_tn_group: null pointer");
// ... 42 lines not shown
```

sgs-gnn_amd/ops.py:

```python
from __future__ import annotations

import ctypes
import os

import numpy as np
import torch

from . import _lib

SAMPLE_LEARNED, SAMPLE_PRIOR = 0, 1
ACT_NONE, ACT_RELU, ACT_RELU_DROPOUT = 0, 1, 2

_workspaces = {}
_retired_workspaces = []
_pin_workspaces = False


def _need_gpu(*tensors):
    for t in tensors:
        if t is not None and not t.is_cuda:
            raise RuntimeError("sgs_gnn_amd: the SGS hot path runs only on a HIP device (got a CPU tensor); "
                               "there is no CPU fallback")


# ... 356 lines not shown
        return values.view_as(values)

    @staticmethod
    def backward(ctx, g):
        (eid,) = ctx.saved_tensors
        act = ctx.active
        if act is not None and act.eid is not None and act.eid.data_ptr() == eid.data_ptr() and act.eid.numel() == eid.numel():
            act.gq = g.contiguous()
            return _zero_token(g.device).expand(ctx.E), None, None, None
        gp = torch.zeros(ctx.E, dtype=g.dtype, device=g.device)
        gp.index_copy_(0, eid, g.contiguous())
        return gp, None, None, None


def select_sampled(probs, eid, values, active=None):
    _need_gpu(probs, eid, values)
    return _SelectSampled.apply(probs, eid, values, active)


def st_weights(p, prior, c, stats, eid):
    _need_gpu(p, prior, stats, eid)
    return _STWeights.apply(p.contiguous(), prior, c, stats, eid)


class Graph:

    def __init__(self, edge_index: torch.Tensor, N: int):
        L = _lib.lib()
        _need_gpu(edge_index)
        if edge_index.dtype != torch.int64 or edge_index.dim() != 2 or edge_index.shape[0] != 2:
            raise RuntimeError("edge_index must be an int64 [2, E] tensor")
        ei = edge_index.contiguous()
        dev = ei.device
        n = ei.shape[1]
        self.edge_index, self.n_edges, self.N = ei, n, int(N)
        ne = max(n, 1)
        sizes = [N + 1, N + 1, ne, ne, ne, ne, max(N, 1)]
        offs = [0]
        for z in sizes:
            offs.append(offs[-1] + ((z + 63) & ~63))
        buf = torch.empty(offs[-1], dtype=torch.int32, device=dev)
        (self.in_ptr, self.out_ptr, self.in_src, self.in_eid, self.out_dst, self.out_eid, self.loop_eid) = (
            buf[offs[i]:offs[i] + sizes[i]] for i in range(7))
        nws = L.sgs_graph_build_workspace_bytes(n, N)
        ws = workspace(nws, dev)
        _lib.check(L.sgs_graph_build(_ptr(ei), n, N, _ptr(self.in_ptr), _ptr(self.in_src), _ptr(self.in_eid),
                                     _ptr(self.out_ptr), _ptr(self.out_dst), _ptr(self.out_eid), _ptr(self.loop_eid),
                                     ws.data_ptr(), ws.numel(), _stream()), "sgs_graph_build")


_SORT_SUBGRAPH_EDGES = int(os.environ.get("SGS_SORT_SUBGRAPH_EDGES", 1 << 22))


def get_subgraph(parent_edge_index: torch.Tensor, N: int, sample, eid=None) -> Graph:
    L = _lib.lib()
    parent = get_graph(parent_edge_index, N)
    ei = sample.edge_index
    n = ei.shape[1]
    g = Graph.__new__(Graph)
    g.edge_index, g.n_edges, g.N = ei, n, int(N)
    ne = max(n, 1)
    sizes = [N + 1, N + 1, ne, ne, ne, ne, max(N, 1)]
    offs = [0]
    for z in sizes:
        offs.append(offs[-1] + ((z + 63) & ~63))
    buf = torch.empty(offs[-1], dtype=torch.int32, device=ei.device)
    (g.in_ptr, g.out_ptr, g.in_src, g.in_eid, g.out_dst, g.out_eid, g.loop_eid) = (buf[offs[i]:offs[i] + sizes[i]] for i in range(7))
    if n >= _SORT_SUBGRAPH_EDGES and src_sorted(parent_edge_index):
        ws = workspace(L.sgs_graph_build_src_sorted_workspace_bytes(n, N), ei.device)
        _lib.check(L.sgs_graph_build_src_sorted(_ptr(ei), n, N, _ptr(g.in_ptr), _ptr(g.in_src), _ptr(g.in_eid), _ptr(g.out_ptr), _ptr(g.out_dst),
                                                _ptr(g.out_eid), _ptr(g.loop_eid), None, ws.data_ptr(), ws.numel(), _stream()),
                   "sgs_graph_build_src_sorted")
        try:
            ei._sgs_graph = g
            ei._sgs_graph_version = ei._version
        except Exception:
            pass
        return g
    ws = workspace(L.sgs_graph_filter_workspace_bytes(parent.n_edges, N), ei.device)
    _lib.check(L.sgs_graph_filter(_ptr(parent.in_ptr), _ptr(parent.in_src), _ptr(parent.in_eid), _ptr(parent.out_ptr), _ptr(parent.out_dst),
                                  _ptr(parent.out_eid), parent.n_edges, N, _ptr(_u8(sample.mask)), _ptr(sample.eid if eid is None else eid, torch.int64), n,
                                  _ptr(g.in_ptr), _ptr(g.in_src), _ptr(g.in_eid), _ptr(g.out_ptr), _ptr(g.out_dst), _ptr(g.out_eid),
                                  _ptr(g.loop_eid), ws.data_ptr(), ws.numel(), _stream()), "sgs_graph_filter")
    try:
        ei._sgs_graph = g
        ei._sgs_graph_version = ei._version
    except Exception:
        pass
    return g


def get_graph(edge_index: torch.Tensor, N: int) -> Graph:
    g = getattr(edge_index, "_sgs_graph", None)
    if g is None or g.N != N or getattr(edge_index, "_sgs_graph_version", -1) != edge_index._version:
        g = Graph(edge_index, N)
        try:
            edge_index._sgs_graph = g
            edge_index._sgs_graph_version = edge_index._version
        except Exception:
            pass
    return g


def get_pairs(edge_index: torch.Tensor, N: int, build: bool = False):
    c = getattr(edge_index, "_sgs_pairs", None)
    if c is not None and c[2] == edge_index._version:
        return c[0], c[1]
    if not build:
        return None
    L = _lib.lib()
    _need_gpu(edge_index)
    g = get_graph(edge_index, N)
    E = g.n_edges
    dev = edge_index.device
    mate = torch.empty(max(E, 1), dtype=torch.int32, device=dev)
    if E > 0:
        ws = workspace(L.sgs_edge_mates_workspace_bytes(E), dev)
        _lib.check(L.sgs_edge_mates(_ptr(g.edge_index), E, N, _ptr(g.out_ptr), _ptr(g.out_dst), _ptr(g.out_eid), _ptr(mate), ws.data_ptr(),
                                    ws.numel(), _stream()), "sgs_edge_mates")
    ar = torch.arange(E, dtype=torch.int32, device=dev)
    canon = ar[(mate[:E] < 0) | (ar < mate[:E])].contiguous()
    try:
        edge_index._sgs_pairs = (canon, mate, edge_index._version)
    except Exception:
        pass
    return canon, mate


class Norm:
    __slots__ = ("graph", "w", "dis", "loopw", "what_in", "what_out", "what_loop", "handle", "_g_first", "_g_extra", "_dw_first", "_park_ok", "__weakref__")


def _norm_forward(graph: Graph, w):
    L = _lib.lib()
    dev = graph.edge_index.device
    nm = Norm()
    nm.graph, nm.w = graph, w
    ne, Nn = max(graph.n_edges, 1), graph.N
    sizes = [Nn, Nn, ne, ne, Nn]
    offs = [0]
    for z in sizes:
        offs.append(offs[-1] + ((z + 63) & ~63))
    buf = torch.empty(offs[-1], dtype=torch.float32, device=dev)
    nm.dis, nm.loopw, nm.what_in, nm.what_out, nm.what_loop = (buf[offs[i]:offs[i] + sizes[i]] for i in range(5))
    nm.handle = None
    _lib.check(L.sgs_gcn_norm_fwd(_ptr(w, torch.float32), graph.n_edges, graph.N, _ptr(graph.in_ptr), _ptr(graph.in_src),
                                  _ptr(graph.in_eid), _ptr(graph.out_ptr), _ptr(graph.out_dst), _ptr(graph.out_eid),
                                  _ptr(graph.loop_eid), _ptr(nm.dis), _ptr(nm.loopw), _ptr(nm.what_in), _ptr(nm.what_out),
                                  _ptr(nm.what_loop), _stream()), "sgs_gcn_norm_fwd")
    return nm


class _GCNNorm(torch.autograd.Function):
    @staticmethod
    def forward(ctx, w, graph, box):
        nm = _norm_forward(graph, w)
        box.append(nm)
        ctx.nm = nm
        return torch.empty(graph.n_edges + graph.N, dtype=torch.float32, device=w.device)

    @staticmethod
    def backward(ctx, g):
        L = _lib.lib()
        nm, gr = ctx.nm, ctx.nm.graph
        g = g.contiguous()
        n = gr.n_edges
        extra = getattr(nm, "_g_extra", None)
        nm._g_first = nm._g_extra = None
        first = getattr(nm, "_dw_first", None)
        first = first() if first is not None else None
        nm._dw_first = None
        if first is not None and (first.numel() != n or not first.is_contiguous() or first.dtype != torch.float32):
            first = None
        dw = first if first is not None else torch.empty(n, dtype=torch.float32, device=g.device)
        if n > 0:
            gw, gl = g[:n], g[n:]
            g2w = g2l = None
            if extra is not None and extra.numel() == g.numel():
                g2w, g2l = extra[:n].data_ptr(), extra[n:].data_ptr()
            elif extra is not None:
                g = g + extra
                gw, gl = g[:n], g[n:]
            nws = L.sgs_gcn_norm_bwd_workspace_bytes(gr.N)
            ws = workspace(nws, g.device)
            _lib.check(L.sgs_gcn_norm_bwd_sum(_ptr(nm.w), gw.data_ptr(), gl.data_ptr(), g2w, g2l, None if first is None else first.data_ptr(), n, gr.N,
                                              _ptr(nm.dis), _ptr(nm.loopw), _ptr(gr.in_ptr), _ptr(gr.in_src), _ptr(gr.in_eid), _ptr(gr.out_ptr),
                                              _ptr(gr.out_dst), _ptr(gr.out_eid), _ptr(gr.loop_eid), _ptr(gr.edge_index), _ptr(dw), ws.data_ptr(),
                                              ws.numel(), _stream()), "sgs_gcn_norm_bwd_sum")
        return (None if first is not None else dw), None, None


def _handle_grad(nm, g):
    if not getattr(nm, "_park_ok", False):
        return g
    if getattr(nm, "_g_first", None) is None:
        nm._g_first = g
        return g
    if getattr(nm, "_g_extra", None) is None:
# ... 304 lines not shown
    return L.sgs_edge_score_get_variant() < 0 and L.sgs_edge_score_get_bwd_variant() < 0


def _edge_score_backward_mask(ctx, L, codes, U, W1, b1, w2, b2, edge_index, eid, graph, n, gp_act, kept=()):
    N, H = codes.shape
    E = edge_index.shape[1]
    dev = codes.device
    f32 = dict(dtype=torch.float32, device=dev)
    p = ctx.p
    bits = torch.empty(n, H // 32, dtype=torch.int32, device=dev)
    dz = torch.empty(n, **f32)
    in_order = eid is None or bool(getattr(ctx.active, "ascending", False))
    if kept and getattr(ctx, "src_sorted", False) and _fused_backward and in_order:
        return _edge_score_backward_fused(ctx, L, codes, U, W1, b1, w2, edge_index, eid, graph, n, gp_act, kept, bits, dz)
    feat = torch.empty(n, H, **f32)
    hdz = Traw = craw = Rraw = None
    if kept:
        maskbits, p_out = kept
        _lib.check(L.sgs_edge_score_bwd_prep(_ptr(codes), N, H, _ptr(edge_index), E, _ptr(eid), n, _ptr(gp_act), _ptr(p_out), _ptr(maskbits),
                                             _ptr(dz), _ptr(bits), _ptr(feat), _stream()), "sgs_edge_score_bwd_prep")
        Traw, craw, Rraw = torch.empty(H, H, **f32), torch.empty(H, **f32), torch.empty(N, H, **f32)
    else:
        tile = L.sgs_edge_score_bwd_tile()
        hdz = torch.empty((n + tile - 1) // tile, H, **f32)
        ws = workspace(L.sgs_edge_score_workspace_bytes(N, H, 0), dev)
        _lib.check(L.sgs_edge_score_bwd_core_bits(_ptr(codes), _ptr(U), N, H, _ptr(edge_index), E, ctx.offset, _ptr(eid), n, _ptr(gp_act), _ptr(W1),
                                                  _ptr(b1), _ptr(w2), _ptr(b2), p, ctx.seed, ctx.site, _ptr(bits), _ptr(hdz), _ptr(dz), _ptr(feat),
                                                  ws.data_ptr(), ws.numel(), _stream()), "sgs_edge_score_bwd_core_bits")
    dfeat = torch.empty(n, H, **f32)
    wsd = workspace(L.sgs_edge_score_workspace_bytes(0, H, 0), dev)
    bf16 = bool(kept) and getattr(ctx, "bf16", False)
    _lib.check((L.sgs_edge_score_bwd_dfeat_bits_bf16 if bf16 else L.sgs_edge_score_bwd_dfeat_bits)(_ptr(bits), _ptr(dz), n, H, _ptr(W1), _ptr(w2), p, _ptr(dfeat), wsd.data_ptr(), wsd.numel(),
                                               _stream()), "sgs_edge_score_bwd_dfeat_bits")
    dW1 = torch.empty_like(W1)
    db1 = torch.empty(H, **f32)
    scale = float(np.float32(1.0) / (np.float32(1.0) - np.float32(p)))
    wsg = workspace(L.sgs_gemm_tn_workspace_bytes(n, H, H), dev)
    db2 = torch.empty(1, **f32)
    _lib.check((L.sgs_gemm_tn_mask_bf16 if bf16 else L.sgs_gemm_tn_mask)(_ptr(bits), _ptr(dz), _ptr(w2), scale, _ptr(feat), n, H, H, _ptr(dW1), 2 * H, _ptr(db1), _ptr(db2), _ptr(Traw),
                                  _ptr(craw), wsg.data_ptr(), wsg.numel(), _stream()), "sgs_gemm_tn_mask")
    dw2 = _colsum(hdz) if hdz is not None else None
    dcodes = torch.empty(N, H, **f32)
    dU = torch.empty(N, H, **f32)
    _lib.check(L.sgs_endpoint_reduce_pair_bits(_ptr(dfeat), _ptr(bits), _ptr(dz), _ptr(w2), p, _ptr(codes), N, H, graph.n_edges, _ptr(graph.in_ptr),
                                               _ptr(graph.in_src), _ptr(graph.in_eid), _ptr(graph.out_ptr), _ptr(graph.out_dst),
                                               _ptr(graph.out_eid), _ptr(dcodes), _ptr(dU), _ptr(Rraw), _stream()), "sgs_endpoint_reduce_pair_bits")
    if dw2 is None:
        dw2 = torch.empty(H, **f32)
        _lib.check(L.sgs_edge_score_dw2_from_parts(_ptr(W1), _ptr(Traw), _ptr(U), _ptr(Rraw), _ptr(b1), _ptr(craw), N, H, p, _ptr(dw2), _stream()),
                   "sgs_edge_score_dw2_from_parts")
    return _edge_score_backward_mask_tail(ctx, L, codes, W1, dcodes, dU, dW1, db1, dw2, db2)


def _edge_score_backward_fused(ctx, L, codes, U, W1, b1, w2, edge_index, eid, graph, n, gp_act, kept, bits, dz):
    N, H = codes.shape
    E = edge_index.shape[1]
    dev = codes.device
    f32 = dict(dtype=torch.float32, device=dev)
    p = ctx.p
    maskbits, p_out = kept
    sd = torch.empty(n, 2, dtype=torch.int32, device=dev)
    wsd = workspace(L.sgs_edge_score_workspace_bytes(0, H, 0), dev)
    bf16 = getattr(ctx, "bf16", False)
    _lib.check((L.sgs_edge_score_bwd_prep_sd_pack_bf16 if bf16 else L.sgs_edge_score_bwd_prep_sd_pack)(_ptr(codes), N, H, _ptr(edge_index), E, _ptr(eid), n, _ptr(gp_act), _ptr(p_out), _ptr(maskbits),
                                                 _ptr(dz), _ptr(bits), _ptr(sd), _ptr(W1), _ptr(w2), p, wsd.data_ptr(), wsd.numel(), _stream()),
               "sgs_edge_score_bwd_prep_sd_pack")
    G = torch.empty(n, H, **f32)
    opart = torch.empty(L.sgs_edge_score_bwd_fused_opart_rows(n, N), H, **f32)
    _lib.check((L.sgs_edge_score_bwd_dfeat_fused_packed_bf16 if bf16 else L.sgs_edge_score_bwd_dfeat_fused_packed)(_ptr(bits), _ptr(dz), _ptr(sd), _ptr(codes), n, N, H, _ptr(G), _ptr(opart), wsd.data_ptr(),
                                                       wsd.numel(), _stream()), "sgs_edge_score_bwd_dfeat_fused_packed")
    dW1 = torch.empty_like(W1)
    db1, db2 = torch.empty(H, **f32), torch.empty(1, **f32)
    Traw, craw, Rraw = torch.empty(H, H, **f32), torch.empty(H, **f32), torch.empty(N, H, **f32)
    scale = float(np.float32(1.0) / (np.float32(1.0) - np.float32(p)))
    wsg = workspace(L.sgs_gemm_tn_workspace_bytes(n, H, H), dev)
    _lib.check((L.sgs_gemm_tn_mask_gather_bf16 if bf16 else L.sgs_gemm_tn_mask_gather)(_ptr(bits), _ptr(dz), _ptr(w2), scale, _ptr(codes), N, _ptr(sd), n, H, H, _ptr(dW1), 2 * H, _ptr(db1), _ptr(db2),
                                         _ptr(Traw), _ptr(craw), wsg.data_ptr(), wsg.numel(), _stream()), "sgs_gemm_tn_mask_gather")
    dcodes, dU = torch.empty(N, H, **f32), torch.empty(N, H, **f32)
    _lib.check(L.sgs_edge_score_bwd_reduce_fused(_ptr(G), _ptr(opart), _ptr(bits), _ptr(dz), _ptr(w2), p, N, H, graph.n_edges, _ptr(graph.in_ptr),
                                                 _ptr(graph.in_eid), _ptr(graph.out_ptr), _ptr(dcodes), _ptr(dU), _ptr(Rraw), _stream()),
               "sgs_edge_score_bwd_reduce_fused")
    dw2 = torch.empty(H, **f32)
    _lib.check(L.sgs_edge_score_dw2_from_parts(_ptr(W1), _ptr(Traw), _ptr(U), _ptr(Rraw), _ptr(b1), _ptr(craw), N, H, p, _ptr(dw2), _stream()),
               "sgs_edge_score_dw2_from_parts")
    return _edge_score_backward_mask_tail(ctx, L, codes, W1, dcodes, dU, dW1, db1, dw2, db2)


def _edge_score_backward_mask_tail(ctx, L, codes, W1, dcodes, dU, dW1, db1, dw2, db2):
    N, H = codes.shape
    dcodes.addmm_(dU, W1[:, H:])
    _leaf_dw(dU, codes, N, H, H, leaf=(ctx, 1), out=dW1, col0=H)
    return dcodes, dW1, db1, dw2, db2, None, None, None, None, None, None, None, None


_EdgeScore._backward_mask = staticmethod(_edge_score_backward_mask)


def edge_score(codes, fc1_w, fc1_b, fc2_w, fc2_b, edge_index, active=None, p=0.0, seed=0, site=0, edge_id_offset=0, pairs="cached",
               precision=None):
    precision = _precision if precision is None else check_precision(precision)
    _need_gpu(codes, fc1_w, edge_index)
    if isinstance(pairs, str):
        pairs = get_pairs(edge_index, codes.shape[0])
    return _EdgeScore.apply(codes.contiguous(), fc1_w.contiguous(), fc1_b.contiguous(), fc2_w.reshape(-1).contiguous(), fc2_b.contiguous(),
                            edge_index.contiguous(), active, float(p), int(seed), int(site), int(edge_id_offset), pairs, precision)


class _EdgeScoreEPD(torch.autograd.Function):

    @staticmethod
    def forward(ctx, A, W1, b1, w2, b2, edge_index, active, p, seed, site, p_ep, seed_x, site_x, seed_y, site_y, edge_id_offset):
        L = _lib.lib()
        N, H = A.shape
        E = edge_index.shape[1]
        out = torch.empty(E, dtype=torch.float32, device=A.device)
        ws = workspace(L.sgs_edge_score_epd_workspace_bytes(H), A.device)
        _lib.check(L.sgs_edge_score_epd_fwd(_ptr(A, torch.float32), N, H, _ptr(edge_index, torch.int64), E, edge_id_offset, _ptr(W1, torch.float32),
                                            _ptr(b1), _ptr(w2), _ptr(b2), float(p), seed, site, float(p_ep), seed_x, site_x, seed_y, site_y, _ptr(out),
                                            ws.data_ptr(), ws.numel(), _stream()), "sgs_edge_score_epd_fwd")
        ctx.save_for_backward(A, W1, b1, w2, b2, edge_index)
        ctx.active, ctx.cfg = active, (float(p), seed, site, float(p_ep), seed_x, site_x, seed_y, site_y, edge_id_offset)
        return out

    @staticmethod
    def backward(ctx, gp):
        L = _lib.lib()
        A, W1, b1, w2, b2, edge_index = ctx.saved_tensors
        p, seed, site, p_ep, seed_x, site_x, seed_y, site_y, offset = ctx.cfg
        N, H = A.shape
        E = edge_index.shape[1]
        dev = A.device
        act = ctx.active
        if act is not None and act.eid is not None:
            eid, graph = act.eid, act.graph
# ... 1604 lines not shown
```

sgs-gnn_amd/training.py:

```python
from __future__ import annotations

import torch
import torch.nn as nn

from . import ops
from .dist import GradSync, is_parallel
from .sampling import cover_graph, cover_nodes, draw_learned, draw_prior, random_edge_sampling
from .utils import segment

_PIPELINES = ("two_pass", "straight_through", "hybrid")


def _fused_ce_ok(criterion) -> bool:
    return (type(criterion) is nn.CrossEntropyLoss and criterion.weight is None and criterion.reduction == "mean"
            and criterion.ignore_index == -100 and getattr(criterion, "label_smoothing", 0.0) == 0.0)


def _ce_spec(criterion):
    if type(criterion) is not nn.CrossEntropyLoss or criterion.reduction != "mean" or criterion.ignore_index != -100:
        return None
    eps = float(getattr(criterion, "label_smoothing", 0.0))
    if not 0.0 <= eps <= 1.0:
        return None
    return criterion.weight, eps


def _ce(criterion, out, batch):
    spec = _ce_spec(criterion)
    if spec is not None:
        return ops.masked_cross_entropy(out, batch.y, batch.train_mask, weight=spec[0], label_smoothing=spec[1])
    return criterion(out[batch.train_mask], batch.y[batch.train_mask])


def _backward(model, loss):
    with segment(model, "backward"), ops.deferred_weight_grads(loss):
        loss.backward()


def _has_train_nodes(batch) -> bool:
    flag = getattr(batch, "_sgs_has_train", None)
    if flag is None:
        flag = bool(batch.train_mask.any())
        try:
            batch._sgs_has_train = flag
        except Exception:
            pass
    return flag


class SampledForward:
    __slots__ = ("rsei", "rs", "edge_probs_full", "smp", "sampled_edge_index", "edge_probs_for_loss", "learned_out",
                 "random_out", "cbuf")


def sampled_prefix(args, batch, q, noise=None):
    if not (args.conditional or args.sparse_edge_mlp):
        return None
    noise = noise or {}
    rs = draw_prior(batch.prob, batch.edge_index, q, noise=noise.get("prior"), cover=cover_graph(args, batch))
    graph_r = ops.get_subgraph(batch.edge_index, batch.x.shape[0], rs)
    ops.gcn_norm(graph_r, None)
    return rs


def _gcn_dual_applies(args, model, batch, ei_learned, ei_random, forked) -> bool:
    from .model import GNNModel
    if not args.conditional or forked or ei_random is None or type(model) is not GNNModel:
        return False
    if not (ops.gcn_dual_enabled() and getattr(args, "sgs_gcn_dual", True)):
        return False
    N = batch.x.shape[0]
    return ops.gcn_dual_ok(ops.get_graph(ei_learned, N), ops.get_graph(ei_random, N), model.gcn1.out_channels, model.gcn2.out_channels)


def sampled_forward(pipeline, args, model, batch, q, use_checkpoint=False, noise=None, side_stream=None, prefix=None,
                    gate_publish=None) -> SampledForward:
    noise = noise or {}
    st = SampledForward()
    N = batch.x.shape[0]
    scorer = model.edge_prob_mlp

    st.rsei, st.rs = None, None
    if args.conditional or args.sparse_edge_mlp:
        rs = prefix if prefix is not None else sampled_prefix(args, batch, q, noise)
        st.rsei, st.rs = rs.edge_index, rs
    st.random_out = None
    forked = side_stream is not None and args.conditional and st.rsei is not None
    if forked:
        ops.gcn_norm(ops.get_graph(st.rsei, N), None)
        main_stream = torch.cuda.current_stream()
        side_stream.wait_stream(main_stream)
        with torch.cuda.stream(side_stream), ops.workspace_slot(2):
            ops.workspace_handover(batch.x.device, slot=2)
            st.random_out = model(batch, st.rsei)

    if pipeline == "two_pass":
        with torch.no_grad():
            st.edge_probs_full = scorer(batch.x, batch.edge_index, st.rsei).squeeze()
    elif pipeline == "hybrid":
        st.edge_probs_full = scorer(batch.x, batch.edge_index, st.rsei, use_checkpoint=use_checkpoint).squeeze()
    else:
        st.edge_probs_full = scorer(batch.x, batch.edge_index, st.rsei).squeeze()
    pass1_active = getattr(scorer, "last_active", None)

    st.smp = smp = draw_learned(batch.prob, st.edge_probs_full, batch.edge_index, q, args.degree_bias_coef,
                                noise=noise.get("sample"), want_p=(pipeline == "hybrid"), cover=cover_graph(args, batch))
    st.sampled_edge_index = smp.edge_index
    graph_s = ops.get_subgraph(batch.edge_index, N, smp)

    if pipeline == "hybrid":
        if pass1_active is not None:
            pass1_active.set(smp.eid, graph_s, ascending=True)
        st.edge_probs_for_loss = ops.select_sampled(st.edge_probs_full, smp.eid, smp.p, pass1_active)
    elif pipeline == "straight_through":
        st.edge_probs_for_loss = ops.st_weights(st.edge_probs_full, batch.prob, args.degree_bias_coef, smp.stats, smp.eid)
    else:
        st.edge_probs_for_loss = scorer(batch.x, smp.edge_index).squeeze()
    if forked:
        main_stream.wait_stream(side_stream)
    if _gcn_dual_applies(args, model, batch, smp.edge_index, st.rsei, forked):
        st.learned_out, st.random_out = model.forward_pair(batch, smp.edge_index, st.edge_probs_for_loss, st.rsei)
    else:
        st.learned_out = model(batch, smp.edge_index, st.edge_probs_for_loss)

    st.cbuf = None
    if args.conditional:
        if st.random_out is None:
            st.random_out = model(batch, st.rsei)
        st.cbuf = ops.gate_counts(st.learned_out, st.random_out, batch.y, batch.train_mask, publish=gate_publish)
    return st


def learned_loss(args, criterion, st: SampledForward, batch):
    c1 = args.regularizer1_coef if args.reg1 == True else 0.0
    c2 = args.consist_reg_coef if args.reg2 == True else 0.0
    spec = _ce_spec(criterion)
    if (c1 != 0.0 or c2 != 0.0) and spec is not None:
        return ops.hybrid_loss(st.learned_out, batch.y, batch.train_mask, st.edge_probs_for_loss, st.sampled_edge_index, c1, c2,
                               weight=spec[0], label_smoothing=spec[1])[0]
    loss = _ce(criterion, st.learned_out, batch)
    if c1 != 0.0 or c2 != 0.0:
        reg, _ = ops.edge_regularizers(st.edge_probs_for_loss, st.learned_out, st.sampled_edge_index, batch.y,
                                       batch.train_mask, c1, c2)
        loss = loss + reg
    return loss


def train(args, epoch, max_epoch, model, optimizer_gnn, optimizer_edge_prob, optimizer, criterion, cluster_loader,
          q=500, alternate_frequency=1):
    pipeline = getattr(args, "pipeline", "two_pass")
    if pipeline not in _PIPELINES:
        pipeline = "two_pass"
    return _train(pipeline, args, epoch, max_epoch, model, optimizer_gnn, optimizer_edge_prob, optimizer, criterion,
                  cluster_loader, q)


def prepare_step_graphs(args, model, optimizer_gnn, optimizer_edge_prob, criterion, cluster_loader, q=500):
    from .stepgraph import StepGraphs
    precision = ops.check_precision(getattr(args, "sgs_precision", None))
    pipeline = getattr(args, "pipeline", "two_pass")
    if pipeline not in _PIPELINES:
# ... 298 lines not shown
```

Baseline: 110.1 million.

## Fuse degree normalization into graph filter and slab reduction into scorer backward

Adds a graph-filter variant that computes GCN degree normalization (dis, loopw) while building the sampled subgraph, so gcn_norm only has to compute edge weights when the cached degree matches the weights. It also splits the masked gather GEMM so its final slab reduction is deferred and run as extra blocks appended to the scorer backward reduce kernel. Both changes remove separate kernel launches and extra passes over graph data. In exchange they add caching keyed on tensor pointer and version, which could go stale, and make the reduce kernel launch larger.

```diff
diff --git a/include/sgs_hip.h b/include/sgs_hip.h
--- a/include/sgs_hip.h
+++ b/include/sgs_hip.h
@@ -84,6 +84,13 @@
                      const int32_t* pout_dst, const int32_t* pout_eid, int64_t E_parent, int64_t N, const uint8_t* mask,
                      const int64_t* sampled_eid, int64_t q, int32_t* in_ptr, int32_t* in_src, int32_t* in_eid, int32_t* out_ptr,
                      int32_t* out_dst, int32_t* out_eid, int32_t* loop_eid, void* ws, size_t ws_bytes, sgs_stream_t stream);
+int sgs_graph_filter_deg_form(int64_t N, int64_t E_parent);
+void sgs_graph_filter_deg_set_form(int form);
+int sgs_graph_filter_deg(const int32_t* pin_ptr, const int32_t* pin_src, const int32_t* pin_eid, const int32_t* pout_ptr,
+                         const int32_t* pout_dst, const int32_t* pout_eid, int64_t E_parent, int64_t N, const uint8_t* mask,
+                         const int64_t* sampled_eid, int64_t q, const float* w, int32_t* in_ptr, int32_t* in_src, int32_t* in_eid,
+                         int32_t* out_ptr, int32_t* out_dst, int32_t* out_eid, int32_t* loop_eid, float* dis, float* loopw, void* ws,
+                         size_t ws_bytes, sgs_stream_t stream);
 
 size_t sgs_graph_build_src_sorted_workspace_bytes(int64_t n_edges, int64_t N);
 int sgs_graph_build_src_sorted(const int64_t* edge_index, int64_t n_edges, int64_t N, int32_t* in_ptr, int32_t* in_src, int32_t* in_eid,
@@ -94,6 +101,9 @@
                      const int32_t* in_eid, const int32_t* out_ptr, const int32_t* out_dst, const int32_t* out_eid,
                      const int32_t* loop_eid, float* dis, float* loopw, float* what_in, float* what_out,
                      float* what_loop, sgs_stream_t stream);
+int sgs_gcn_norm_weights(const float* w, int64_t n_edges, int64_t N, const int32_t* in_ptr, const int32_t* in_src, const int32_t* in_eid,
+                         const int32_t* out_ptr, const int32_t* out_dst, const int32_t* out_eid, const float* dis, const float* loopw,
+                         float* what_in, float* what_out, float* what_loop, sgs_stream_t stream);
 
 int sgs_gcn_degree_partial(const float* w, int64_t n_edges, int64_t N, const int32_t* in_ptr, const int32_t* in_src,
                            const int32_t* in_eid, float* degpart, sgs_stream_t stream);
@@ -290,6 +300,33 @@
 int sgs_gemm_tn_mask_gather_bf16(const uint32_t* Abits, const float* dz, const float* rowscale, float scale, const float* codes, int64_t codes_rows,
                                  const int32_t* sd, int64_t K, int64_t M, int64_t N, float* C, int64_t ldc, float* colsum_A, float* dz_sum, float* C_raw,
                                  float* colsum_raw, void* ws, size_t ws_bytes, sgs_stream_t stream);
+
+typedef struct SgsGemmTnPending {
+    const float* slab;
+    const float* colsum_rows;
+    const float* dz_parts;
+    const float* rowscale;
+    float* C;
+    float* colsum_A;
+    float* dz_sum;
+    float* C_raw;
+    float* colsum_raw;
+    int64_t M, N, ldc;
+    int32_t n_slabs;
+    int32_t csplit;
+    int32_t n_dz_parts;
+    float scale;
+} SgsGemmTnPending;
+int sgs_gemm_tn_mask_gather_slabs(const uint32_t* Abits, const float* dz, const float* rowscale, float scale, const float* codes, int64_t codes_rows,
+                                  const int32_t* sd, int64_t K, int64_t M, int64_t N, float* C, int64_t ldc, float* colsum_A, float* dz_sum,
+                                  float* C_raw, float* colsum_raw, SgsGemmTnPending* pending, void* ws, size_t ws_bytes, sgs_stream_t stream);
+int sgs_gemm_tn_mask_gather_slabs_bf16(const uint32_t* Abits, const float* dz, const float* rowscale, float scale, const float* codes,
+                                       int64_t codes_rows, const int32_t* sd, int64_t K, int64_t M, int64_t N, float* C, int64_t ldc,
+                                       float* colsum_A, float* dz_sum, float* C_raw, float* colsum_raw, SgsGemmTnPending* pending, void* ws,
+                                       size_t ws_bytes, sgs_stream_t stream);
+int sgs_scorer_bwd_reduce_tail(const float* G, const float* opart, const uint32_t* dvbits, const float* dz, const float* w2, float p_drop,
+                               int64_t N, int64_t H, int64_t nnz, const int32_t* in_ptr, const int32_t* in_eid, const int32_t* out_ptr,
+                               float* out_codes, float* out_U, float* out_U_raw, const SgsGemmTnPending* pending, sgs_stream_t stream);
 
 int sgs_endpoint_reduce(const float* M_out, const float* M_in, const float* T, int64_t N, int64_t H, int64_t nnz,
                         const int32_t* in_ptr, const int32_t* in_src, const int32_t* in_eid, const int32_t* out_ptr,
diff --git a/sgs-gnn_amd/csrc/edge_score.hip b/sgs-gnn_amd/csrc/edge_score.hip
--- a/sgs-gnn_amd/csrc/edge_score.hip
+++ b/sgs-gnn_amd/csrc/edge_score.hip
@@ -2,6 +2,7 @@
 
 #include "sgs_common.h"
 #include "endpoint_reduce.h"
+#include "slab_reduce.h"
 
 namespace sgs {
 namespace {
@@ -1846,15 +1847,14 @@
 }
 
 template <int NW>
-__global__ void __launch_bounds__(64 * NW) scorer_bwd_reduce(const float* __restrict__ G, const float* __restrict__ opart,
-                                                            const uint32_t* __restrict__ bits, const float* __restrict__ dz,
-                                                            const float* __restrict__ w2, float scale, int64_t N, int64_t H,
-                                                            const int* __restrict__ in_ptr, const int* __restrict__ in_eid,
-                                                            const int* __restrict__ out_ptr, float* __restrict__ out_codes,
-                                                            float* __restrict__ out_U, float* __restrict__ out_Uraw) {
+__device__ __forceinline__ void scorer_bwd_reduce_body(const int64_t v, const float* __restrict__ G, const float* __restrict__ opart,
+                                                       const uint32_t* __restrict__ bits, const float* __restrict__ dz,
+                                                       const float* __restrict__ w2, float scale, int64_t N, int64_t H,
+                                                       const int* __restrict__ in_ptr, const int* __restrict__ in_eid,
+                                                       const int* __restrict__ out_ptr, float* __restrict__ out_codes,
+                                                       float* __restrict__ out_U, float* __restrict__ out_Uraw) {
     __shared__ float part[2][NW][256];
     const int lane = threadIdx.x & 63, wave = threadIdx.x >> 6;
-    const int64_t v = blockIdx.x;
     const int ob = out_ptr[v], no = out_ptr[v + 1] - ob;
     const int ib = in_ptr[v], ni = in_ptr[v + 1] - ib;
     const int w0 = ob >> 5, np = no > 0 ? ((ob + no - 1) >> 5) - w0 + 1 : 0;
@@ -1944,6 +1944,29 @@
         }
         __syncthreads();
     }
+}
+template <int NW>
+__global__ void __launch_bounds__(64 * NW) scorer_bwd_reduce(const float* __restrict__ G, const float* __restrict__ opart,
+                                                            const uint32_t* __restrict__ bits, const float* __restrict__ dz,
+                                                            const float* __restrict__ w2, float scale, int64_t N, int64_t H,
+                                                            const int* __restrict__ in_ptr, const int* __restrict__ in_eid,
+                                                            const int* __restrict__ out_ptr, float* __restrict__ out_codes,
+                                                            float* __restrict__ out_U, float* __restrict__ out_Uraw) {
+    scorer_bwd_reduce_body<NW>(blockIdx.x, G, opart, bits, dz, w2, scale, N, H, in_ptr, in_eid, out_ptr, out_codes, out_U, out_Uraw);
+}
+template <int NW>
+__global__ void __launch_bounds__(64 * NW) scorer_bwd_reduce_tail(const float* __restrict__ G, const float* __restrict__ opart,
+                                                                 const uint32_t* __restrict__ bits, const float* __restrict__ dz,
+                                                                 const float* __restrict__ w2, float scale, int64_t N, int64_t H,
+                                                                 const int* __restrict__ in_ptr, const int* __restrict__ in_eid,
+                                                                 const int* __restrict__ out_ptr, float* __restrict__ out_codes,
+                                                                 float* __restrict__ out_U, float* __restrict__ out_Uraw, SgsGemmTnPending red) {
+    if (static_cast<int64_t>(blockIdx.x) >= N) {
+        const int64_t i = (static_cast<int64_t>(blockIdx.x) - N) * (64 * NW) + threadIdx.x;
+        if (i < gemm_tn_reduce_threads(red)) gemm_tn_reduce_elem(i, red);
+        return;
+    }
+    scorer_bwd_reduce_body<NW>(blockIdx.x, G, opart, bits, dz, w2, scale, N, H, in_ptr, in_eid, out_ptr, out_codes, out_U, out_Uraw);
 }
 
 __global__ void __launch_bounds__(256) epd_endpoint_reduce(const float* __restrict__ dfeat2, const float* __restrict__ A, int64_t N, int64_t H,
@@ -2620,6 +2643,36 @@
     return SGS_OK;
 }
 
+int sgs_scorer_bwd_reduce_tail(const float* G, const float* opart, const uint32_t* dvbits, const float* dz, const float* w2, float p_drop,
+                               int64_t N, int64_t H, int64_t nnz, const int32_t* in_ptr, const int32_t* in_eid, const int32_t* out_ptr,
+                               float* out_codes, float* out_U, float* out_U_raw, const SgsGemmTnPending* pending, sgs_stream_t stream_) {
+    hipStream_t stream = static_cast<hipStream_t>(stream_);
+    SGS_REQUIRE(N >= 0 && H >= 0 && H % 32 == 0 && N < (int64_t(1) << 31) && p_drop >= 0.f && p_drop < 1.f, SGS_EINVAL,
+                "sgs_scorer_bwd_reduce_tail: needs H %% 32 == 0");
+    SGS_REQUIRE(pending, SGS_EINVAL, "sgs_scorer_bwd_reduce_tail: null pointer");
+    const SgsGemmTnPending& r = *pending;
+    SGS_REQUIRE(r.M >= 0 && r.N >= 0 && r.M < (1 << 30) && r.N < (1 << 30) && r.n_slabs >= 0 && r.csplit >= 0 && r.n_dz_parts >= 0 &&
+                    (r.M * r.N == 0 || (r.slab && r.C && r.ldc >= r.N)) && (!r.colsum_A || r.colsum_rows) && (!r.colsum_raw || r.colsum_A) &&
+                    (!r.dz_sum || r.dz_parts),
+                SGS_EINVAL, "sgs_scorer_bwd_reduce_tail: bad pending reduction");
+    if (N == 0 || H == 0) {
+        SGS_REQUIRE(r.M * r.N == 0, SGS_EINVAL, "sgs_scorer_bwd_reduce_tail: a pending reduction needs N > 0 and H > 0");
+        return SGS_OK;
+    }
+    SGS_REQUIRE(G && opart && dvbits && dz && w2 && in_ptr && in_eid && out_ptr && out_codes && out_U, SGS_EINVAL,
+                "sgs_scorer_bwd_reduce_tail: null pointer");
+    const float scale = 1.0f / (1.0f - p_drop);
+    const int64_t threads = gemm_tn_reduce_threads(r);
+    if (nnz >= 64 * N)
+        hipLaunchKernelGGL((scorer_bwd_reduce_tail<16>), dim3(static_cast<unsigned>(N + cdiv(threads, 1024))), dim3(1024), 0, stream, G, opart, dvbits,
+                           dz, w2, scale, N, H, in_ptr, in_eid, out_ptr, out_codes, out_U, out_U_raw, r);
+    else
+        hipLaunchKernelGGL((scorer_bwd_reduce_tail<4>), dim3(static_cast<unsigned>(N + cdiv(threads, 256))), dim3(256), 0, stream, G, opart, dvbits, dz,
+                           w2, scale, N, H, in_ptr, in_eid, out_ptr, out_codes, out_U, out_U_raw, r);
+    SGS_LAUNCH_OK();
+    return SGS_OK;
+}
+
 int sgs_edge_score_dw2_from_parts(const float* W1, const float* T_raw, const float* U, const float* R_raw, const float* b1, const float* c_raw,
                                   int64_t N, int64_t H, float p_drop, float* dw2, sgs_stream_t stream_) {
     hipStream_t stream = static_cast<hipStream_t>(stream_);
diff --git a/sgs-gnn_amd/csrc/gcn.hip b/sgs-gnn_amd/csrc/gcn.hip
--- a/sgs-gnn_amd/csrc/gcn.hip
+++ b/sgs-gnn_amd/csrc/gcn.hip
@@ -289,8 +289,42 @@
 }
 
 constexpr int64_t kSelfScanRows = 4096;
+template <bool BITS>
+__device__ __forceinline__ int filter_fill_span(int b, int e, int w, int64_t row, bool out, const int* __restrict__ peid, const int* __restrict__ pcol,
+                                                const uint8_t* __restrict__ mask, const int* __restrict__ pos, int* __restrict__ ccol,
+                                                int* __restrict__ ceid, int& loop) {
+    const int lane = threadIdx.x & 63;
+    int pe_c = 0, col_c = 0;
+    if (e > b) { const int kc = min(b + lane, e - 1); pe_c = peid[kc]; col_c = pcol[kc]; }
+    for (int k0 = b; k0 < e; k0 += 64) {
+        const int k = k0 + lane;
+        const int kn = min(k + 64, e - 1);
+        const int pe_n = peid[kn], col_n = pcol[kn];
+        const bool m_c = mask_at<BITS>(mask, pe_c);
+        const bool sel = k < e && m_c;
+        const int ne = sel ? pos[pe_c] : 0;
+        const int col = col_c;
+        pe_c = pe_n; col_c = col_n;
+        const unsigned long long bal = __ballot(sel);
+        if (sel) {
+            const int o = w + __popcll(bal & ((1ull << lane) - 1ull));
+            ccol[o] = col;
+            ceid[o] = ne;
+        }
+        if (!out) {
+            const unsigned long long lb = __ballot(sel && col == static_cast<int>(row));
+            if (lb) loop = __shfl(ne, 63 - __clzll(lb), 64);
+        }
+        w += __popcll(bal);
+    }
+    return w;
+}
+struct FilledRow {
+    int64_t row;
+    int b, e, loop;
+};
 template <bool BITS, bool SCAN>
-__device__ __forceinline__ void filter_fill_body(int64_t nrows, const int* __restrict__ pin_ptr, const int* __restrict__ pin_src, const int* __restrict__ pin_eid,
+__device__ __forceinline__ FilledRow filter_fill_body(int64_t nrows, const int* __restrict__ pin_ptr, const int* __restrict__ pin_src, const int* __restrict__ pin_eid,
                                                  const int* __restrict__ pout_ptr, const int* __restrict__ pout_dst,
                                                  const int* __restrict__ pout_eid, int64_t N, const uint8_t* __restrict__ mask,
                                                  const int* __restrict__ pos, int* __restrict__ in_ptr, int* __restrict__ in_src,
@@ -299,7 +333,7 @@
                                                  const int* __restrict__ cnt_out) {
     const int lane = threadIdx.x & 63;
     const int64_t r = (static_cast<int64_t>(blockIdx.x) * kT + threadIdx.x) >> 6;
-    if (r >= nrows) return;
+    if (r >= nrows) return FilledRow{-1, 0, 0, -1};
     const bool out = r >= N;
     const int64_t row = out ? r - N : r;
     const int* pptr = out ? pout_ptr : pin_ptr;
@@ -322,31 +356,10 @@
         w = (out ? out_ptr : in_ptr)[row];
     }
     int loop = -1;
-    const int b = pptr[row], e = pptr[row + 1];
-    int pe_c = 0, col_c = 0;
-    if (e > b) { const int kc = min(b + lane, e - 1); pe_c = peid[kc]; col_c = pcol[kc]; }
-    for (int k0 = b; k0 < e; k0 += 64) {
-        const int k = k0 + lane;
-        const int kn = min(k + 64, e - 1);
-        const int pe_n = peid[kn], col_n = pcol[kn];
-        const bool m_c = mask_at<BITS>(mask, pe_c);
-        const bool sel = k < e && m_c;
-        const int ne = sel ? pos[pe_c] : 0;
-        const int col = col_c;
-        pe_c = pe_n; col_c = col_n;
-        const unsigned long long bal = __ballot(sel);
-        if (sel) {
-            const int o = w + __popcll(bal & ((1ull << lane) - 1ull));
-            ccol[o] = col;
-            ceid[o] = ne;
-        }
-        if (!out) {
-            const unsigned long long lb = __ballot(sel && col == static_cast<int>(row));
-            if (lb) loop = __shfl(ne, 63 - __clzll(lb), 64);
-        }
-        w += __popcll(bal);
-    }
+    const int w_first = w;
+    w = filter_fill_span<BITS>(pptr[row], pptr[row + 1], w, row, out, peid, pcol, mask, pos, ccol, ceid, loop);
     if (!out && lane == 0) loop_eid[row] = loop;
+    return FilledRow{out ? -1 : row, w_first, w, loop};
 }
 template <bool BITS, bool SCAN = false>
 __global__ void __launch_bounds__(kT) filter_fill(const int* __restrict__ pin_ptr, const int* __restrict__ pin_src, const int* __restrict__ pin_eid,
@@ -360,31 +373,114 @@
                                  out_dst, out_eid, loop_eid, cnt_in, cnt_out);
 }
 
-__device__ __forceinline__ void norm_deg_body(const float* __restrict__ w, int64_t N, const int* __restrict__ in_ptr,
-                                              const int* __restrict__ in_src, const int* __restrict__ in_eid,
-                                              const int* __restrict__ loop_eid, float* __restrict__ dis,
-                                              float* __restrict__ loopw) {
+template <int U = 1>
+__device__ __forceinline__ void norm_deg_row(const float* __restrict__ w, int64_t i, int b, int e, const int* in_src, const int* in_eid, int le,
+                                             float* __restrict__ dis, float* __restrict__ loopw) {
     const int lane = threadIdx.x & 63;
-    const int64_t i = (static_cast<int64_t>(blockIdx.x) * kT + threadIdx.x) >> 6;
-    if (i >= N) return;
-    const int b = in_ptr[i], e = in_ptr[i + 1];
     float acc = 0.f;
-    for (int k = b + lane; k < e; k += 64) {
-        if (in_src[k] != static_cast<int>(i)) acc += w ? w[in_eid[k]] : 1.0f;
+    if constexpr (U == 1) {
+        for (int k = b + lane; k < e; k += 64) {
+            if (in_src[k] != static_cast<int>(i)) acc += w ? w[in_eid[k]] : 1.0f;
+        }
+    } else {
+        for (int k0 = b + lane; k0 - lane < e; k0 += 64 * U) {
+            int s[U], id[U];
+            float v[U];
+#pragma unroll
+            for (int u = 0; u < U; ++u) {
+                const int k = min(k0 + 64 * u, e - 1);
+                s[u] = in_src[k];
+                id[u] = w ? in_eid[k] : 0;
+            }
+#pragma unroll
+            for (int u = 0; u < U; ++u) v[u] = w ? w[id[u]] : 1.0f;
+#pragma unroll
+            for (int u = 0; u < U; ++u)
+                if (k0 + 64 * u < e && s[u] != static_cast<int>(i)) acc += v[u];
+        }
     }
     acc = wave_sum_all(acc);
-    const int le = loop_eid[i];
     const float lw = (le >= 0 && w) ? w[le] : 1.0f;
     const float deg = lw + acc;
     float di = 1.0f / sqrtf(deg);
     if (isinf(di)) di = 0.f;
     if (lane == 0) { dis[i] = di; loopw[i] = lw; }
 }
+__device__ __forceinline__ void norm_deg_body(const float* __restrict__ w, int64_t N, const int* __restrict__ in_ptr,
+                                              const int* __restrict__ in_src, const int* __restrict__ in_eid,
+                                              const int* __restrict__ loop_eid, float* __restrict__ dis,
+                                              float* __restrict__ loopw) {
+    const int64_t i = (static_cast<int64_t>(blockIdx.x) * kT + threadIdx.x) >> 6;
+    if (i >= N) return;
+    norm_deg_row(w, i, in_ptr[i], in_ptr[i + 1], in_src, in_eid, loop_eid[i], dis, loopw);
+}
 __global__ void __launch_bounds__(kT) norm_deg(const float* __restrict__ w, int64_t N, const int* __restrict__ in_ptr,
                                               const int* __restrict__ in_src, const int* __restrict__ in_eid,
                                               const int* __restrict__ loop_eid, float* __restrict__ dis,
                                               float* __restrict__ loopw) {
     norm_deg_body(w, N, in_ptr, in_src, in_eid, loop_eid, dis, loopw);
+}
+__global__ void __launch_bounds__(kT) filter_fill_deg(const int* __restrict__ pin_ptr, const int* __restrict__ pin_src, const int* __restrict__ pin_eid,
+                                                     const int* __restrict__ pout_ptr, const int* __restrict__ pout_dst,
+                                                     const int* __restrict__ pout_eid, int64_t N, const uint8_t* __restrict__ mask,
+                                                     const int* __restrict__ pos, int* in_ptr, int* in_src, int* in_eid, int* out_ptr, int* out_dst,
+                                                     int* out_eid, int* loop_eid, const int* __restrict__ cnt_in, const int* __restrict__ cnt_out,
+                                                     const float* __restrict__ w, float* __restrict__ dis, float* __restrict__ loopw) {
+    const FilledRow fr = filter_fill_body<false, true>(2 * N, pin_ptr, pin_src, pin_eid, pout_ptr, pout_dst, pout_eid, N, mask, pos, in_ptr, in_src,
+                                                       in_eid, out_ptr, out_dst, out_eid, loop_eid, cnt_in, cnt_out);
+    __syncthreads();
+    if (fr.row >= 0) norm_deg_row<8>(w, fr.row, fr.b, fr.e, in_src, in_eid, fr.loop, dis, loopw);
+}
+__global__ void __launch_bounds__(kT) filter_fill_deg_wg(const int* __restrict__ pin_ptr, const int* __restrict__ pin_src,
+                                                        const int* __restrict__ pin_eid, const int* __restrict__ pout_ptr,
+                                                        const int* __restrict__ pout_dst, const int* __restrict__ pout_eid, int64_t N,
+                                                        const uint8_t* __restrict__ mask, const int* __restrict__ pos, int* in_ptr, int* in_src,
+                                                        int* in_eid, int* out_ptr, int* out_dst, int* out_eid, int* loop_eid,
+                                                        const int* __restrict__ cnt_in, const int* __restrict__ cnt_out,
+                                                        const float* __restrict__ w, float* __restrict__ dis, float* __restrict__ loopw) {
+    __shared__ int s_cnt[4], s_loop[4];
+    const int lane = threadIdx.x & 63, wave = threadIdx.x >> 6;
+    const int64_t r = blockIdx.x;
+    const bool out = r >= N;
+    const int64_t row = out ? r - N : r;
+    const int* pptr = out ? pout_ptr : pin_ptr;
+    const int* pcol = out ? pout_dst : pin_src;
+    const int* peid = out ? pout_eid : pin_eid;
+    const int* cnt = out ? cnt_out : cnt_in;
+    int acc = 0;
+    for (int64_t i = lane; i < row; i += 64) acc += cnt[i];
+    const int w0 = wave_sum_int_all(acc);
+    if (threadIdx.x == 0) {
+        int* cptr = out ? out_ptr : in_ptr;
+        cptr[row] = w0;
+        if (row == N - 1) cptr[N] = w0 + cnt[row];
+    }
+    const int b = pptr[row], e = pptr[row + 1];
+    const int chunk = ((e - b + 255) >> 8) << 6;
+    const int qb = min(e, b + wave * chunk), qe = min(e, qb + chunk);
+    int c = 0;
+    for (int k = qb + lane; k - lane < qe; k += 256) {
+        int id[4];
+#pragma unroll
+        for (int u = 0; u < 4; ++u) id[u] = peid[min(k + 64 * u, qe - 1)];
+#pragma unroll
+        for (int u = 0; u < 4; ++u) c += (k + 64 * u < qe && mask[id[u]] != 0) ? 1 : 0;
+    }
+    c = wave_sum_int_all(c);
+    if (lane == 0) s_cnt[wave] = c;
+    __syncthreads();
+    int cur = w0;
+    for (int j = 0; j < wave; ++j) cur += s_cnt[j];
+    int loop = -1;
+    filter_fill_span<false>(qb, qe, cur, row, out, peid, pcol, mask, pos, out ? out_dst : in_src, out ? out_eid : in_eid, loop);
+    if (lane == 0) s_loop[wave] = loop;
+    __syncthreads();
+    if (out || wave != 0) return;
+    loop = -1;
+#pragma unroll
+    for (int j = 0; j < 4; ++j) loop = s_loop[j] >= 0 ? s_loop[j] : loop;
+    if (lane == 0) loop_eid[row] = loop;
+    norm_deg_row<8>(w, row, w0, w0 + ((s_cnt[0] + s_cnt[1]) + (s_cnt[2] + s_cnt[3])), in_src, in_eid, loop, dis, loopw);
 }
 
 __global__ void __launch_bounds__(kT) deg_partial(const float* __restrict__ w, int64_t N, const int* __restrict__ in_ptr,
@@ -1443,6 +1539,57 @@
     return SGS_OK;
 }
 
+static int g_filter_deg_form = -1;
+void sgs_graph_filter_deg_set_form(int form) { g_filter_deg_form = (form == 1 || form == 4) ? form : -1; }
+int sgs_graph_filter_deg_form(int64_t N, int64_t E_parent) {
+    if (!(E_parent >= 0 && E_parent < (int64_t(1) << 23) && N > 0 && N <= kSelfScanRows)) return 0;
+    if (g_filter_deg_form > 0) return g_filter_deg_form;
+    return E_parent >= 128 * N ? 4 : 1;
+}
+
+int sgs_graph_filter_deg(const int32_t* pin_ptr, const int32_t* pin_src, const int32_t* pin_eid, const int32_t* pout_ptr,
+                         const int32_t* pout_dst, const int32_t* pout_eid, int64_t E_parent, int64_t N, const uint8_t* mask,
+                         const int64_t* sampled_eid, int64_t q, const float* w, int32_t* in_ptr, int32_t* in_src, int32_t* in_eid,
+                         int32_t* out_ptr, int32_t* out_dst, int32_t* out_eid, int32_t* loop_eid, float* dis, float* loopw, void* ws,
+                         size_t ws_bytes, sgs_stream_t stream_) {
+    hipStream_t stream = static_cast<hipStream_t>(stream_);
+    SGS_REQUIRE(N <= 0 || (dis && loopw), SGS_EINVAL, "sgs_graph_filter_deg: null pointer");
+    const int form = sgs_graph_filter_deg_form(N, E_parent);
+    if (form == 0) {
+        if (int rc = sgs_graph_filter(pin_ptr, pin_src, pin_eid, pout_ptr, pout_dst, pout_eid, E_parent, N, mask, sampled_eid, q, in_ptr, in_src,
+                                      in_eid, out_ptr, out_dst, out_eid, loop_eid, ws, ws_bytes, stream_))
+            return rc;
+        if (N == 0) return SGS_OK;
+        hipLaunchKernelGGL(norm_deg, dim3(cdiv(N * 64, kT)), dim3(kT), 0, stream, w, N, in_ptr, in_src, in_eid, loop_eid, dis, loopw);
+        SGS_LAUNCH_OK();
+        return SGS_OK;
+    }
+    SGS_REQUIRE(q >= 0 && q <= E_parent, SGS_EINVAL, "sgs_graph_filter_deg: bad sizes");
+    SGS_REQUIRE(pin_ptr && pout_ptr && in_ptr && out_ptr && loop_eid && (E_parent == 0 || (pin_src && pin_eid && pout_dst && pout_eid && mask)) &&
+                    (q == 0 || (sampled_eid && in_src && in_eid && out_dst && out_eid)), SGS_EINVAL, "sgs_graph_filter_deg: null pointer");
+    SGS_REQUIRE(ws && ws_bytes >= sgs_graph_filter_workspace_bytes(E_parent, N), SGS_EWORKSPACE, "sgs_graph_filter_deg: workspace too small");
+    Carver cv(ws);
+    int* cnt_in = cv.take<int>(N + 1);
+    int* cnt_out = cv.take<int>(N + 1);
+    cv.take<int>(N + 1);
+    cv.take<int>(N + 1);
+    int* pos = cv.take<int>(E_parent + 1);
+    const int64_t n_row_blocks = cdiv(2 * N * 64, kT);
+    const dim3 g1(static_cast<unsigned>(n_row_blocks + cdiv(q, kT))), g3(static_cast<unsigned>(n_row_blocks)), blk(kT);
+    hipLaunchKernelGGL(filter_count_scatter<false>, g1, blk, 0, stream, pin_ptr, pin_eid, pout_ptr, pout_eid, N, mask, sampled_eid, q, n_row_blocks,
+                       cnt_in, cnt_out, pos);
+    if (form == 4)
+        hipLaunchKernelGGL(filter_fill_deg_wg, dim3(static_cast<unsigned>(2 * N)), blk, 0, stream, pin_ptr, pin_src, pin_eid, pout_ptr, pout_dst,
+                           pout_eid, N, mask, static_cast<const int*>(pos), in_ptr, in_src, in_eid, out_ptr, out_dst, out_eid, loop_eid,
+                           static_cast<const int*>(cnt_in), static_cast<const int*>(cnt_out), w, dis, loopw);
+    else
+        hipLaunchKernelGGL(filter_fill_deg, g3, blk, 0, stream, pin_ptr, pin_src, pin_eid, pout_ptr, pout_dst, pout_eid, N, mask,
+                           static_cast<const int*>(pos), in_ptr, in_src, in_eid, out_ptr, out_dst, out_eid, loop_eid,
+                           static_cast<const int*>(cnt_in), static_cast<const int*>(cnt_out), w, dis, loopw);
+    SGS_LAUNCH_OK();
+    return SGS_OK;
+}
+
 size_t sgs_edge_mates_workspace_bytes(int64_t n_edges) { return carve_bytes(n_edges < 0 ? 0 : n_edges, 4) + 256; }
 
 int sgs_edge_mates(const int64_t* edge_index, int64_t n_edges, int64_t N, const int32_t* out_ptr, const int32_t* out_dst,
@@ -1472,6 +1619,19 @@
     hipLaunchKernelGGL(norm_deg, dim3(cdiv(N * 64, kT)), dim3(kT), 0, stream, w, N, in_ptr, in_src, in_eid, loop_eid, dis, loopw);
     hipLaunchKernelGGL(norm_weights, dim3(cdiv(2 * N * 64, kT)), dim3(kT), 0, stream, w, N, n_edges, in_ptr, in_src, in_eid,
                        out_ptr, out_dst, out_eid, dis, loopw, what_in, what_out, what_loop);
+    SGS_LAUNCH_OK();
+    return SGS_OK;
+}
+
+int sgs_gcn_norm_weights(const float* w, int64_t n_edges, int64_t N, const int32_t* in_ptr, const int32_t* in_src, const int32_t* in_eid,
+                         const int32_t* out_ptr, const int32_t* out_dst, const int32_t* out_eid, const float* dis, const float* loopw,
+                         float* what_in, float* what_out, float* what_loop, sgs_stream_t stream_) {
+    hipStream_t stream = static_cast<hipStream_t>(stream_);
+    SGS_REQUIRE(N >= 0 && n_edges >= 0, SGS_EINVAL, "sgs_gcn_norm_weights: bad sizes");
+    if (N == 0) return SGS_OK;
+    SGS_REQUIRE(in_ptr && out_ptr && dis && loopw && what_loop, SGS_EINVAL, "sgs_gcn_norm_weights: null pointer");
+    hipLaunchKernelGGL(norm_weights, dim3(cdiv(2 * N * 64, kT)), dim3(kT), 0, stream, w, N, n_edges, in_ptr, in_src, in_eid, out_ptr, out_dst,
+                       out_eid, dis, loopw, what_in, what_out, what_loop);
     SGS_LAUNCH_OK();
     return SGS_OK;
 }
diff --git a/sgs-gnn_amd/csrc/gemm_tn.hip b/sgs-gnn_amd/csrc/gemm_tn.hip
--- a/sgs-gnn_amd/csrc/gemm_tn.hip
+++ b/sgs-gnn_amd/csrc/gemm_tn.hip
@@ -1,4 +1,5 @@
 #include "sgs_common.h"
+#include "slab_reduce.h"
 
 namespace sgs {
 namespace {
@@ -129,55 +130,8 @@
                                                       float scale = 1.f, const float* __restrict__ dzpart = nullptr, int nz = 0,
                                                       float* __restrict__ dzsum = nullptr, float* __restrict__ Craw = nullptr,
                                                       float* __restrict__ csraw = nullptr, int csplit = 0) {
-    const int64_t i = static_cast<int64_t>(blockIdx.x) * 256 + threadIdx.x;
-    if (i >= mn) {
-        const int64_t c = i - mn;
-        if (dzsum && c == M) {
-            float acc = 0.f;
-            for (int z = 0; z < nz; ++z) acc += dzpart[z];
-            dzsum[0] = acc;
-        }
-        if (colsum && c < M) {
-            float acc = 0.f;
-            const int ncs = csplit > 0 ? csplit : ksplit;
-            if (csplit > 0) {
-                float a8[8] = {0.f, 0.f, 0.f, 0.f, 0.f, 0.f, 0.f, 0.f};
-                int s = 0;
-                for (; s + 8 <= ncs; s += 8) {
-                    float v[8];
-#pragma unroll
-                    for (int j = 0; j < 8; ++j) v[j] = cpart[static_cast<int64_t>(s + j) * M + c];
-#pragma unroll
-                    for (int j = 0; j < 8; ++j) a8[j] += v[j];
-                }
-                for (; s < ncs; ++s) a8[0] += cpart[static_cast<int64_t>(s) * M + c];
-                acc = ((a8[0] + a8[1]) + (a8[2] + a8[3])) + ((a8[4] + a8[5]) + (a8[6] + a8[7]));
-            } else
-            for (int s = 0; s < ncs; ++s) acc += cpart[static_cast<int64_t>(s) * M + c];
-            if (csraw) csraw[c] = acc;
-            colsum[c] = rowscale ? acc * (rowscale[c] * scale) : acc;
-        }
-        return;
-    }
-    float acc = 0.f;
-    if (csplit > 0) {
-        float a8[8] = {0.f, 0.f, 0.f, 0.f, 0.f, 0.f, 0.f, 0.f};
-        int s = 0;
-        for (; s + 8 <= ksplit; s += 8) {
-            float v[8];
-#pragma unroll
-            for (int j = 0; j < 8; ++j) v[j] = slab[static_cast<int64_t>(s + j) * mn + i];
-#pragma unroll
-            for (int j = 0; j < 8; ++j) a8[j] += v[j];
-        }
-        for (; s < ksplit; ++s) a8[0] += slab[static_cast<int64_t>(s) * mn + i];
-        acc = ((a8[0] + a8[1]) + (a8[2] + a8[3])) + ((a8[4] + a8[5]) + (a8[6] + a8[7]));
-    } else
-    for (int s = 0; s < ksplit; ++s) acc += slab[static_cast<int64_t>(s) * mn + i];
-    if (Craw) Craw[i] = acc;
-    if (rowscale) acc *= rowscale[i / N] * scale;
-    if (ldc > 0 && ldc != N) C[(i / N) * ldc + (i % N)] = acc;
-    else C[i] = acc;
+    gemm_tn_reduce_elem(static_cast<int64_t>(blockIdx.x) * 256 + threadIdx.x, slab, mn, ksplit, C, cpart, M, colsum, N, ldc, rowscale, scale, dzpart,
+                        nz, dzsum, Craw, csraw, csplit);
 }
 
 constexpr int kTallK = 8192;
@@ -817,7 +771,7 @@
 static int gemm_tn_impl(const float* A, const float* B, int64_t K, int64_t M, int64_t N, float* C, float* colsum_A, void* ws,
                         size_t ws_bytes, hipStream_t stream, int64_t ldc = 0, const uint32_t* Abits = nullptr, const float* dz = nullptr,
                         const float* rowscale = nullptr, float scale = 1.f, float* dz_sum = nullptr, float* C_raw = nullptr,
-                        float* colsum_raw = nullptr, const int32_t* sd = nullptr, bool one = false);
+                        float* colsum_raw = nullptr, const int32_t* sd = nullptr, bool one = false, SgsGemmTnPending* pending = nullptr);
 static int g_tall_bf16x6 = 1;
 static int g_gather_shared = 1, g_gather_slabs = 0;
 void sgs_gemm_tn_set_gather_variant(int shared, int slabs) { g_gather_shared = shared ? 1 : 0; g_gather_slabs = slabs > 0 ? slabs : 0; }
@@ -897,9 +851,38 @@
                         dz_sum, C_raw, colsum_raw, sd, true);
 }
 
+static int mask_gather_slabs(const char* who, bool one, const uint32_t* Abits, const float* dz, const float* rowscale, float scale, const float* codes,
+                             int64_t codes_rows, const int32_t* sd, int64_t K, int64_t M, int64_t N, float* C, int64_t ldc, float* colsum_A,
+                             float* dz_sum, float* C_raw, float* colsum_raw, SgsGemmTnPending* pending, void* ws, size_t ws_bytes,
+                             sgs_stream_t stream_) {
+    if (pending) *pending = SgsGemmTnPending{};
+    SGS_REQUIRE(ldc >= N, SGS_EINVAL, "%s: ldc < N", who);
+    SGS_REQUIRE(codes_rows > 0 && codes_rows * N < (int64_t(1) << 32), SGS_EINVAL, "%s: the codes table needs 32-bit element offsets", who);
+    SGS_REQUIRE(Abits && dz && rowscale && codes && sd && pending, SGS_EINVAL, "%s: null pointer", who);
+    SGS_REQUIRE(sgs_gemm_tn_mask_supported(K, M, N), SGS_EINVAL, "%s: shape not served (check sgs_gemm_tn_mask_supported)", who);
+    SGS_REQUIRE(!colsum_raw || colsum_A, SGS_EINVAL, "%s: colsum_raw needs colsum_A", who);
+    return gemm_tn_impl(nullptr, codes, K, M, N, C, colsum_A, ws, ws_bytes, static_cast<hipStream_t>(stream_), ldc, Abits, dz, rowscale, scale,
+                        dz_sum, C_raw, colsum_raw, sd, one, pending);
+}
+
+int sgs_gemm_tn_mask_gather_slabs(const uint32_t* Abits, const float* dz, const float* rowscale, float scale, const float* codes, int64_t codes_rows,
+                                  const int32_t* sd, int64_t K, int64_t M, int64_t N, float* C, int64_t ldc, float* colsum_A, float* dz_sum,
+                                  float* C_raw, float* colsum_raw, SgsGemmTnPending* pending, void* ws, size_t ws_bytes, sgs_stream_t stream_) {
+    return mask_gather_slabs("sgs_gemm_tn_mask_gather_slabs", false, Abits, dz, rowscale, scale, codes, codes_rows, sd, K, M, N, C, ldc, colsum_A,
+                             dz_sum, C_raw, colsum_raw, pending, ws, ws_bytes, stream_);
+}
+
+int sgs_gemm_tn_mask_gather_slabs_bf16(const uint32_t* Abits, const float* dz, const float* rowscale, float scale, const float* codes,
+                                       int64_t codes_rows, const int32_t* sd, int64_t K, int64_t M, int64_t N, float* C, int64_t ldc,
+                                       float* colsum_A, float* dz_sum, float* C_raw, float* colsum_raw, SgsGemmTnPending* pending, void* ws,
+                                       size_t ws_bytes, sgs_stream_t stream_) {
+    return mask_gather_slabs("sgs_gemm_tn_mask_gather_slabs_bf16", true, Abits, dz, rowscale, scale, codes, codes_rows, sd, K, M, N, C, ldc,
+                             colsum_A, dz_sum, C_raw, colsum_raw, pending, ws, ws_bytes, stream_);
+}
+
 static int gemm_tn_impl(const float* A, const float* B, int64_t K, int64_t M, int64_t N, float* C, float* colsum_A, void* ws,
                         size_t ws_bytes, hipStream_t stream, int64_t ldc, const uint32_t* Abits, const float* dz, const float* rowscale,
-                        float scale, float* dz_sum, float* C_raw, float* colsum_raw, const int32_t* sd, bool one) {
+                        float scale, float* dz_sum, float* C_raw, float* colsum_raw, const int32_t* sd, bool one, SgsGemmTnPending* pending) {
     SGS_REQUIRE(K >= 0 && M >= 0 && N >= 0 && M < (1 << 30) && N < (1 << 30), SGS_EINVAL, "sgs_gemm_tn: bad sizes");
     if (M == 0 || N == 0) return SGS_OK;
     SGS_REQUIRE(C && (K == 0 || ((A || Abits) && B)), SGS_EINVAL, "sgs_gemm_tn: null pointer");
@@ -946,6 +929,10 @@
                 if (NGc == 1) SGS_MASKFEAT(1, 1); else if (NGc == 2) SGS_MASKFEAT(1, 2); else if (NGc == 4) SGS_MASKFEAT(1, 4); else SGS_MASKFEAT(1, 8);
             }
 #undef SGS_MASKFEAT
+            if (pending)
+                *pending = SgsGemmTnPending{slab, colsum_A ? cpart2 : nullptr, dzp, rowscale, C, colsum_A, dz_sum, C_raw, colsum_raw, M, N,
+                                            ldc > 0 ? ldc : N, ns, ns * NGc, ns, scale};
+            else
             hipLaunchKernelGGL(gemm_tn_reduce, dim3(cdiv(M * N + M + 1, 256)), dim3(256), 0, stream, slab, M * N, ns, C,
                                static_cast<const float*>(colsum_A ? cpart2 : nullptr), static_cast<int>(M), colsum_A, static_cast<int>(N),
                                ldc > 0 ? ldc : N, rowscale, scale, static_cast<const float*>(dzp), ns, dz_sum, C_raw, colsum_raw, ns * NGc);
@@ -983,6 +970,10 @@
         hipLaunchKernelGGL((gemm_tn_tall_bf16x6<NW, true>), dim3(cdiv(M, 128), cdiv(N, 64), n_slabs), dim3(64 * NW), lds, stream, A, B, K,
                            static_cast<int>(M), static_cast<int>(N), ks, slab, (colsum_A || dz_sum) ? cpart : static_cast<float*>(nullptr), Abits, dz,
                            dzpart);
+        if (pending)
+            *pending = SgsGemmTnPending{slab, colsum_A ? cpart : nullptr, dzpart, rowscale, C, colsum_A, dz_sum, C_raw, colsum_raw, M, N,
+                                        ldc > 0 ? ldc : N, n_slabs, 0, ks, scale};
+        else
         hipLaunchKernelGGL(gemm_tn_reduce, dim3(cdiv(M * N + M + 1, 256)), dim3(256), 0, stream, slab, M * N, n_slabs, C,
                            static_cast<const float*>(colsum_A ? cpart : nullptr), static_cast<int>(M), colsum_A, static_cast<int>(N),
                            ldc > 0 ? ldc : N, rowscale, scale, static_cast<const float*>(dzpart), ks, dz_sum, C_raw, colsum_raw);
diff --git a/sgs-gnn_amd/csrc/slab_reduce.h b/sgs-gnn_amd/csrc/slab_reduce.h
--- /dev/null
+++ b/sgs-gnn_amd/csrc/slab_reduce.h
@@ -0,0 +1,66 @@
+#pragma once
+#include "sgs_common.h"
+
+namespace sgs {
+
+__device__ __forceinline__ void gemm_tn_reduce_elem(int64_t i, const float* __restrict__ slab, int64_t mn, int ksplit, float* __restrict__ C,
+                                                    const float* __restrict__ cpart, int M, float* __restrict__ colsum, int N, int64_t ldc,
+                                                    const float* __restrict__ rowscale, float scale, const float* __restrict__ dzpart, int nz,
+                                                    float* __restrict__ dzsum, float* __restrict__ Craw, float* __restrict__ csraw, int csplit) {
+    if (i >= mn) {
+        const int64_t c = i - mn;
+        if (dzsum && c == M) {
+            float acc = 0.f;
+            for (int z = 0; z < nz; ++z) acc += dzpart[z];
+            dzsum[0] = acc;
+        }
+        if (colsum && c < M) {
+            float acc = 0.f;
+            const int ncs = csplit > 0 ? csplit : ksplit;
+            if (csplit > 0) {
+                float a8[8] = {0.f, 0.f, 0.f, 0.f, 0.f, 0.f, 0.f, 0.f};
+                int s = 0;
+                for (; s + 8 <= ncs; s += 8) {
+                    float v[8];
+#pragma unroll
+                    for (int j = 0; j < 8; ++j) v[j] = cpart[static_cast<int64_t>(s + j) * M + c];
+#pragma unroll
+                    for (int j = 0; j < 8; ++j) a8[j] += v[j];
+                }
+                for (; s < ncs; ++s) a8[0] += cpart[static_cast<int64_t>(s) * M + c];
+                acc = ((a8[0] + a8[1]) + (a8[2] + a8[3])) + ((a8[4] + a8[5]) + (a8[6] + a8[7]));
+            } else
+            for (int s = 0; s < ncs; ++s) acc += cpart[static_cast<int64_t>(s) * M + c];
+            if (csraw) csraw[c] = acc;
+            colsum[c] = rowscale ? acc * (rowscale[c] * scale) : acc;
+        }
+        return;
+    }
+    float acc = 0.f;
+    if (csplit > 0) {
+        float a8[8] = {0.f, 0.f, 0.f, 0.f, 0.f, 0.f, 0.f, 0.f};
+        int s = 0;
+        for (; s + 8 <= ksplit; s += 8) {
+            float v[8];
+#pragma unroll
+            for (int j = 0; j < 8; ++j) v[j] = slab[static_cast<int64_t>(s + j) * mn + i];
+#pragma unroll
+            for (int j = 0; j < 8; ++j) a8[j] += v[j];
+        }
+        for (; s < ksplit; ++s) a8[0] += slab[static_cast<int64_t>(s) * mn + i];
+        acc = ((a8[0] + a8[1]) + (a8[2] + a8[3])) + ((a8[4] + a8[5]) + (a8[6] + a8[7]));
+    } else
+    for (int s = 0; s < ksplit; ++s) acc += slab[static_cast<int64_t>(s) * mn + i];
+    if (Craw) Craw[i] = acc;
+    if (rowscale) acc *= rowscale[i / N] * scale;
+    if (ldc > 0 && ldc != N) C[(i / N) * ldc + (i % N)] = acc;
+    else C[i] = acc;
+}
+
+__device__ __forceinline__ void gemm_tn_reduce_elem(int64_t i, const SgsGemmTnPending& r) {
+    gemm_tn_reduce_elem(i, r.slab, r.M * r.N, r.n_slabs, r.C, r.colsum_rows, static_cast<int>(r.M), r.colsum_A, static_cast<int>(r.N), r.ldc,
+                        r.rowscale, r.scale, r.dz_parts, r.n_dz_parts, r.dz_sum, r.C_raw, r.colsum_raw, r.csplit);
+}
+__host__ __device__ __forceinline__ int64_t gemm_tn_reduce_threads(const SgsGemmTnPending& r) { return r.M * r.N + r.M + 1; }
+
+}
diff --git a/sgs-gnn_amd/ops.py b/sgs-gnn_amd/ops.py
--- a/sgs-gnn_amd/ops.py
+++ b/sgs-gnn_amd/ops.py
@@ -432,7 +432,21 @@
 _SORT_SUBGRAPH_EDGES = int(os.environ.get("SGS_SORT_SUBGRAPH_EDGES", 1 << 22))
 
 
-def get_subgraph(parent_edge_index: torch.Tensor, N: int, sample, eid=None) -> Graph:
+class _UnitWeights:
+    def __repr__(self):
+        return "UNIT_WEIGHTS"
+
+
+UNIT_WEIGHTS = _UnitWeights()
+
+
+def _weights_key(w):
+    if w is None or w is UNIT_WEIGHTS:
+        return UNIT_WEIGHTS
+    return (w.data_ptr(), w._version, w.numel())
+
+
+def get_subgraph(parent_edge_index: torch.Tensor, N: int, sample, eid=None, w=None) -> Graph:
     L = _lib.lib()
     parent = get_graph(parent_edge_index, N)
     ei = sample.edge_index
@@ -458,10 +472,26 @@
             pass
         return g
     ws = workspace(L.sgs_graph_filter_workspace_bytes(parent.n_edges, N), ei.device)
-    _lib.check(L.sgs_graph_filter(_ptr(parent.in_ptr), _ptr(parent.in_src), _ptr(parent.in_eid), _ptr(parent.out_ptr), _ptr(parent.out_dst),
-                                  _ptr(parent.out_eid), parent.n_edges, N, _ptr(_u8(sample.mask)), _ptr(sample.eid if eid is None else eid, torch.int64), n,
-                                  _ptr(g.in_ptr), _ptr(g.in_src), _ptr(g.in_eid), _ptr(g.out_ptr), _ptr(g.out_dst), _ptr(g.out_eid),
-                                  _ptr(g.loop_eid), ws.data_ptr(), ws.numel(), _stream()), "sgs_graph_filter")
+    if w is not None:
+        wt = None if w is UNIT_WEIGHTS else w
+        if wt is not None:
+            _need_gpu(wt)
+            if wt.dtype != torch.float32 or wt.numel() != n or not wt.is_contiguous():
+                raise RuntimeError(f"get_subgraph: w must be a contiguous float32 [{n}] tensor or UNIT_WEIGHTS")
+        pad = (max(N, 1) + 63) & ~63
+        deg = torch.empty(2 * pad, dtype=torch.float32, device=ei.device)
+        dis, loopw = deg[:N], deg[pad:pad + N]
+        _lib.check(L.sgs_graph_filter_deg(_ptr(parent.in_ptr), _ptr(parent.in_src), _ptr(parent.in_eid), _ptr(parent.out_ptr), _ptr(parent.out_dst),
+                                          _ptr(parent.out_eid), parent.n_edges, N, _ptr(_u8(sample.mask)),
+                                          _ptr(sample.eid if eid is None else eid, torch.int64), n, _ptr(wt, torch.float32), _ptr(g.in_ptr),
+                                          _ptr(g.in_src), _ptr(g.in_eid), _ptr(g.out_ptr), _ptr(g.out_dst), _ptr(g.out_eid), _ptr(g.loop_eid),
+                                          _ptr(dis), _ptr(loopw), ws.data_ptr(), ws.numel(), _stream()), "sgs_graph_filter_deg")
+        g._deg = (dis, loopw, _weights_key(w))
+    else:
+        _lib.check(L.sgs_graph_filter(_ptr(parent.in_ptr), _ptr(parent.in_src), _ptr(parent.in_eid), _ptr(parent.out_ptr), _ptr(parent.out_dst),
+                                      _ptr(parent.out_eid), parent.n_edges, N, _ptr(_u8(sample.mask)), _ptr(sample.eid if eid is None else eid, torch.int64), n,
+                                      _ptr(g.in_ptr), _ptr(g.in_src), _ptr(g.in_eid), _ptr(g.out_ptr), _ptr(g.out_dst), _ptr(g.out_eid),
+                                      _ptr(g.loop_eid), ws.data_ptr(), ws.numel(), _stream()), "sgs_graph_filter")
     try:
         ei._sgs_graph = g
         ei._sgs_graph_version = ei._version
@@ -517,13 +547,27 @@
     nm = Norm()
     nm.graph, nm.w = graph, w
     ne, Nn = max(graph.n_edges, 1), graph.N
+    nm.handle = None
+    deg = getattr(graph, "_deg", None)
+    if deg is not None and deg[2] == _weights_key(w):
+        sizes = [ne, ne, Nn]
+        offs = [0]
+        for z in sizes:
+            offs.append(offs[-1] + ((z + 63) & ~63))
+        buf = torch.empty(offs[-1], dtype=torch.float32, device=dev)
+        nm.dis, nm.loopw = deg[0], deg[1]
+        nm.what_in, nm.what_out, nm.what_loop = (buf[offs[i]:offs[i] + sizes[i]] for i in range(3))
+        _lib.check(L.sgs_gcn_norm_weights(_ptr(w, torch.float32), graph.n_edges, graph.N, _ptr(graph.in_ptr), _ptr(graph.in_src),
+                                          _ptr(graph.in_eid), _ptr(graph.out_ptr), _ptr(graph.out_dst), _ptr(graph.out_eid), _ptr(nm.dis),
+                                          _ptr(nm.loopw), _ptr(nm.what_in), _ptr(nm.what_out), _ptr(nm.what_loop), _stream()),
+                   "sgs_gcn_norm_weights")
+        return nm
     sizes = [Nn, Nn, ne, ne, Nn]
     offs = [0]
     for z in sizes:
         offs.append(offs[-1] + ((z + 63) & ~63))
     buf = torch.empty(offs[-1], dtype=torch.float32, device=dev)
     nm.dis, nm.loopw, nm.what_in, nm.what_out, nm.what_loop = (buf[offs[i]:offs[i] + sizes[i]] for i in range(5))
-    nm.handle = None
     _lib.check(L.sgs_gcn_norm_fwd(_ptr(w, torch.float32), graph.n_edges, graph.N, _ptr(graph.in_ptr), _ptr(graph.in_src),
                                   _ptr(graph.in_eid), _ptr(graph.out_ptr), _ptr(graph.out_dst), _ptr(graph.out_eid),
                                   _ptr(graph.loop_eid), _ptr(nm.dis), _ptr(nm.loopw), _ptr(nm.what_in), _ptr(nm.what_out),
@@ -934,6 +978,12 @@
     return _edge_score_backward_mask_tail(ctx, L, codes, W1, dcodes, dU, dW1, db1, dw2, db2)
 
 
+class GemmTnPending(ctypes.Structure):
+    _fields_ = ([(n, ctypes.c_void_p) for n in ("slab", "colsum_rows", "dz_parts", "rowscale", "C", "colsum_A", "dz_sum", "C_raw", "colsum_raw")]
+                + [(n, ctypes.c_int64) for n in ("M", "N", "ldc")] + [(n, ctypes.c_int32) for n in ("n_slabs", "csplit", "n_dz_parts")]
+                + [("scale", ctypes.c_float)])
+
+
 def _edge_score_backward_fused(ctx, L, codes, U, W1, b1, w2, edge_index, eid, graph, n, gp_act, kept, bits, dz):
     N, H = codes.shape
     E = edge_index.shape[1]
@@ -956,12 +1006,14 @@
     Traw, craw, Rraw = torch.empty(H, H, **f32), torch.empty(H, **f32), torch.empty(N, H, **f32)
     scale = float(np.float32(1.0) / (np.float32(1.0) - np.float32(p)))
     wsg = workspace(L.sgs_gemm_tn_workspace_bytes(n, H, H), dev)
-    _lib.check((L.sgs_gemm_tn_mask_gather_bf16 if bf16 else L.sgs_gemm_tn_mask_gather)(_ptr(bits), _ptr(dz), _ptr(w2), scale, _ptr(codes), N, _ptr(sd), n, H, H, _ptr(dW1), 2 * H, _ptr(db1), _ptr(db2),
-                                         _ptr(Traw), _ptr(craw), wsg.data_ptr(), wsg.numel(), _stream()), "sgs_gemm_tn_mask_gather")
+    pending = GemmTnPending()
+    _lib.check((L.sgs_gemm_tn_mask_gather_slabs_bf16 if bf16 else L.sgs_gemm_tn_mask_gather_slabs)(
+        _ptr(bits), _ptr(dz), _ptr(w2), scale, _ptr(codes), N, _ptr(sd), n, H, H, _ptr(dW1), 2 * H, _ptr(db1), _ptr(db2), _ptr(Traw), _ptr(craw),
+        ctypes.addressof(pending), wsg.data_ptr(), wsg.numel(), _stream()), "sgs_gemm_tn_mask_gather_slabs")
     dcodes, dU = torch.empty(N, H, **f32), torch.empty(N, H, **f32)
-    _lib.check(L.sgs_edge_score_bwd_reduce_fused(_ptr(G), _ptr(opart), _ptr(bits), _ptr(dz), _ptr(w2), p, N, H, graph.n_edges, _ptr(graph.in_ptr),
-                                                 _ptr(graph.in_eid), _ptr(graph.out_ptr), _ptr(dcodes), _ptr(dU), _ptr(Rraw), _stream()),
-               "sgs_edge_score_bwd_reduce_fused")
+    _lib.check(L.sgs_scorer_bwd_reduce_tail(_ptr(G), _ptr(opart), _ptr(bits), _ptr(dz), _ptr(w2), p, N, H, graph.n_edges, _ptr(graph.in_ptr),
+                                            _ptr(graph.in_eid), _ptr(graph.out_ptr), _ptr(dcodes), _ptr(dU), _ptr(Rraw), ctypes.addressof(pending),
+                                            _stream()), "sgs_scorer_bwd_reduce_tail")
     dw2 = torch.empty(H, **f32)
     _lib.check(L.sgs_edge_score_dw2_from_parts(_ptr(W1), _ptr(Traw), _ptr(U), _ptr(Rraw), _ptr(b1), _ptr(craw), N, H, p, _ptr(dw2), _stream()),
                "sgs_edge_score_dw2_from_parts")
diff --git a/sgs-gnn_amd/training.py b/sgs-gnn_amd/training.py
--- a/sgs-gnn_amd/training.py
+++ b/sgs-gnn_amd/training.py
@@ -58,7 +58,7 @@
         return None
     noise = noise or {}
     rs = draw_prior(batch.prob, batch.edge_index, q, noise=noise.get("prior"), cover=cover_graph(args, batch))
-    graph_r = ops.get_subgraph(batch.edge_index, batch.x.shape[0], rs)
+    graph_r = ops.get_subgraph(batch.edge_index, batch.x.shape[0], rs, w=ops.UNIT_WEIGHTS)
     ops.gcn_norm(graph_r, None)
     return rs
 
@@ -106,7 +106,7 @@
     st.smp = smp = draw_learned(batch.prob, st.edge_probs_full, batch.edge_index, q, args.degree_bias_coef,
                                 noise=noise.get("sample"), want_p=(pipeline == "hybrid"), cover=cover_graph(args, batch))
     st.sampled_edge_index = smp.edge_index
-    graph_s = ops.get_subgraph(batch.edge_index, N, smp)
+    graph_s = ops.get_subgraph(batch.edge_index, N, smp, w=smp.p if pipeline == "hybrid" else None)
 
     if pipeline == "hybrid":
         if pass1_active is not None:
```

Result: faster. 112.1 million, median of 6 (+1.8%).
